# Rikorose/DeepFilterNet

Hardware: NVIDIA H100
Metric: 48kHz audio-sec/sec (batched enhance) (higher is better)
Workload: dtype f32 (bf16x3 tensor-core contractions, fp32 accumulate; DSP and gates IEEE fp32)

## Files before the change

deepfilternet_b200/csrc/dfb_common.cuh:

```cuda
#pragma once
#include <cuda_runtime.h>
#include <stdint.h>

#include <atomic>
#include <cstdarg>
#include <cstdio>
#include <mutex>
#include <string>
#include <vector>

#include "../../include/dfb200.h"

namespace dfb {

extern thread_local std::string g_err;
extern std::atomic<int64_t> g_launches;

inline int fail(int code, const char *fmt, ...) {
    char buf[512];
    va_list ap;
    va_start(ap, fmt);
    vsnprintf(buf, sizeof buf, fmt, ap);
    va_end(ap);
    g_err = buf;
    return code;
}

#define DFB_CUDA(expr)                                                                          \
    do {                                                                                        \
        cudaError_t e__ = (expr);                                                               \
        if (e__ != cudaSuccess)                                                                 \
            return dfb::fail(DFB_ERR_CUDA, "%s failed: %s (%s:%d)", #expr, cudaGetErrorString(e__), \
                             __FILE__, __LINE__);                                               \
    } while (0)

#define DFB_LAUNCH_CHECK()                                                                      \
    do {                                                                                        \
        dfb::g_launches.fetch_add(1, std::memory_order_relaxed);                                \
        cudaError_t e__ = cudaGetLastError();                                                   \
        if (e__ != cudaSuccess)                                                                 \
            return dfb::fail(DFB_ERR_CUDA, "kernel launch failed: %s (%s:%d)",                  \
                             cudaGetErrorString(e__), __FILE__, __LINE__);                      \
    } while (0)

struct ProfScope {
    int slot = -1;
    cudaStream_t s;
    ProfScope(const char *name, cudaStream_t stream);
    ~ProfScope();
};
#define DFB_PROF(name, stream) dfb::ProfScope prof_scope__(name, stream)

struct PerDeviceOnce {
    std::mutex mu;
    std::atomic<unsigned long long> done{0};
    struct Guard {
        std::unique_lock<std::mutex> lk;
        PerDeviceOnce *o = nullptr;
        unsigned long long bit = 0;
        Guard() = default;
        Guard(Guard &&g) noexcept : lk(std::move(g.lk)), o(g.o), bit(g.bit) {}
        explicit operator bool() const { return lk.owns_lock(); }
        ~Guard() { if (lk.owns_lock()) o->done.fetch_or(bit, std::memory_order_release); }
    };
    Guard first() {
        int d = 0;
        cudaGetDevice(&d);
        const unsigned long long bit = 1ull << (d & 63);
        Guard g;
        if (done.load(std::memory_order_acquire) & bit) return g;
        g.lk = std::unique_lock<std::mutex>(mu);
        if (done.load(std::memory_order_acquire) & bit) { g.lk.unlock(); g.lk.release(); return g; }
        g.o = this; g.bit = bit;
        return g;
    }
};

int use_device(int device);

struct Arena {
    char *base = nullptr;
    size_t cap = 0, off = 0;
    int reserve(size_t bytes);
    void reset() { off = 0; }
    template <typename T>
    T *take(size_t n) {
        size_t b = (n * sizeof(T) + 255) & ~size_t(255);
        if (off + b > cap) return nullptr;
        T *p = reinterpret_cast<T *>(base + off);
        off += b;
        return p;
    }
    void release();
};

constexpr int kMaxErb = 64;

struct DspTables {
    const float *window;
    const float2 *tw_a_fwd;
    const float2 *tw_a_inv;
    const float2 *tw960;
    const int *erb_off;
    const float *erb_kinv;
    const unsigned char *band_of_bin;
    float wnorm;
    int fft, hop, F, E;
};

struct RaggedRow { int64_t in_off, len, out_off, out_len, Tf; };

struct LinkRow { int first, n; };
enum { kReduceNone = 0, kReduceMax = 1, kReduceMean = 2 };
struct SlotCtl { float lim, beta, lim0, beta0; int64_t sw; };

__device__ __forceinline__ int stream_first(const int64_t *first, int b, int64_t w0) {
    if (!first) return 0;
    const int64_t d = first[b] - w0;
    return d > 0 ? (int)d : 0;
}

__device__ __forceinline__ float erb_norm_init(int j, int E) {
    return (E == 1) ? -60.f : __fadd_rn(-60.f, __fmul_rn((float)j, __fdiv_rn(-30.f, (float)(E - 1))));
}
__device__ __forceinline__ float unit_norm_init(int k, int Fd) {
    return (Fd == 1) ? 0.001f : __fadd_rn(0.001f, __fmul_rn((float)k, __fdiv_rn(__fsub_rn(0.0001f, 0.001f), (float)(Fd - 1))));
}

struct ApplyParams {
    const float2 *spec;
    const float *m;
    const float *coefs;
    float *audio;
    float2 *spec_out;
    int64_t out_stride;
    int64_t out_offset;
    int64_t out_len;
    int Tf, mode, nb_df, order, lookahead;
    int spec_T, Tv, t_first;
    int mc_T;
    int frames_per_warp;
    int pf, mask_only;
    float pf_beta;
    const float *lsnr;
    float th_min, th_erb, th_df;
    const float *alpha;
    float atten_lim;
    const float *init_tail;
    float *final_tail;
    int carry;
    const RaggedRow *rows;
    int64_t w0;
    int t_emit;
    const int64_t *first;
    const LinkRow *links;
    int reduce;
};

}

struct dfb_state;
namespace dfb {
struct AnaWindow { int t_begin, nf, out_t0, Tbuf; int64_t row_stride; const RaggedRow *rows = nullptr; };
int launch_analysis(dfb_state *st, const float *d_audio, int64_t C, int64_t T, float *d_spec, float *d_erb_db,
                    cudaStream_t s, const float *d_init_mem = nullptr, const AnaWindow *w = nullptr);
int launch_feat_norm(const float *d_erb, int E, int64_t erb_stride, const float *d_spec, int Fd, int64_t spec_stride,
                     int64_t C, int64_t Tf, float alpha, const float *d_erb_state, const float *d_unit_state,
                     float *d_feat_erb, float *d_feat_spec, cudaStream_t s, int64_t Ts = 0, float *d_erb_state_out = nullptr,
                     float *d_unit_state_out = nullptr, bool ref_bits = false);
int launch_apply_synthesis(dfb_state *st, const ApplyParams &p, int64_t B, cudaStream_t s, const SlotCtl *ctl = nullptr);
struct GruWindow { const float *h0; float *hT; int t0, Ts; const int64_t *first = nullptr; int64_t w0 = 0;  };
int launch_gru_tc(cudaStream_t s, const float *xproj, const float *whh, const float *bhh, const float *res, float *hout,
                  unsigned short *hout_hi, unsigned short *hout_lo, int B, int T, long long *dbg = nullptr, int wide = 0,
                  int planes_res = 0, const GruWindow *w = nullptr, int H = 256);
int launch_gemm_bf16x3(cudaStream_t s, const void *x_hi, const void *x_lo, int64_t ldx, const void *w_hi, const void *w_lo,
                       const float *bias, float *y, int64_t ldy, int64_t M, int N, int K);
int launch_gl_bx(cudaStream_t s, const unsigned short *x_hi, const unsigned short *x_lo, int64_t ldx, const float *w_img,
                 const float *res, int64_t ldr, float *y, int64_t ldy, unsigned short *y_hi, unsigned short *y_lo, int64_t ldp,
                 int64_t M, int G, int Ig, int Hg, int act, float oscale, float ooffset);
bool gl_bx_geometry(int G, int Ig, int Hg, int *gpc_out, int *hgp_out, int *stages_out);
int launch_df_convp_tc(cudaStream_t s, const float *c0, const float *w_sw, const float *w2, const float *bias, float *coefs, int B, int T,
                       int Fd, const int64_t *first = nullptr, int64_t w0 = 0);
int launch_to_planes(cudaStream_t s, const float *x, int64_t ldx, int64_t M, int K, unsigned short *hi, unsigned short *lo);
}

struct dfb_state {
    int device, sr, fft, hop, nb_erb, min_nb_erb_freqs;
    std::vector<int64_t> erb;
    std::vector<float> window;
    void *d_tables = nullptr;
    dfb::DspTables tb{};
    dfb::Arena arena;
    cudaStream_t stream = nullptr;
    std::vector<float> analysis_mem, synthesis_mem;
};
```

deepfilternet_b200/csrc/dfb_gl.cu:

```cuda
#include <cuda.h>
#include <cuda_bf16.h>

#include <map>
#include <mutex>
#include <tuple>

#include "dfb_common.cuh"
#include "dfb_ptx.cuh"

namespace dfb {

constexpr int kGxThreads = 288, kGxMaxStages = 6, kGxBoxBytes = 128 * 128 ;
constexpr int kGxMaxChunks = 16;

struct GlBxParams {
    const unsigned short *w_img;
    const float *res; int64_t ldr;
    float *y; int64_t ldy;
    unsigned short *y_hi, *y_lo; int64_t ldp;
    int M, G, Ig, Hg, Hgp, gpc, act, stages;
    float oscale, ooffset;
};

__device__ __forceinline__ float gx_act(float x, int act) {
    if (act == 1) return fmaxf(x, 0.f);
    if (act == 2) return gt_tanh(x);
    return x;
}

__device__ __noinline__ void gl_store_chunk(const GlBxParams &p, int c, int g0, int cpg, int64_t mrow, int lane, float a00, float a01,
                                            float a02, float a03, float a10, float a11, float a12, float a13) {
    const float a[2][4] = {{a00, a01, a02, a03}, {a10, a11, a12, a13}};
    const int gl = c / cpg;
#pragma unroll
    for (int j = 0; j < 2; j++) {
        const int n = (c - gl * cpg) * 16 + j * 8 + 2 * (lane & 3);
        if (n >= p.Hg) continue;
        const int64_t col = (int64_t)(g0 + gl) * p.Hg + n;
        float2 rv[2];
#pragma unroll
        for (int h = 0; h < 2; h++) {
            const int64_t m = mrow + 8 * h;
            rv[h] = (p.res && m < p.M) ? *reinterpret_cast<const float2 *>(p.res + m * p.ldr + col) : make_float2(0.f, 0.f);
        }
#pragma unroll
        for (int h = 0; h < 2; h++) {
            const int64_t m = mrow + 8 * h;
            if (m >= p.M) continue;
            float2 x;
            x.x = gx_act(a[j][2 * h], p.act) * p.oscale + p.ooffset + rv[h].x;
            x.y = gx_act(a[j][2 * h + 1], p.act) * p.oscale + p.ooffset + rv[h].y;
            if (p.y) *reinterpret_cast<float2 *>(p.y + m * p.ldy + col) = x;
            if (p.y_hi) {
                uint32_t hv, lv;
                bf16x2_split(x.x, x.y, hv, lv);
                *reinterpret_cast<uint32_t *>(p.y_hi + m * p.ldp + col) = hv;
                *reinterpret_cast<uint32_t *>(p.y_lo + m * p.ldp + col) = lv;
            }
        }
    }
}

__global__ void __launch_bounds__(kGxThreads, 1)
k_gl_bx(const __grid_constant__ CUtensorMap tmXhi, const __grid_constant__ CUtensorMap tmXlo, const __grid_constant__ GlBxParams p) {
    extern __shared__ __align__(1024) unsigned char gx_smem_raw[];
    const uint32_t sb = (smem_u32(gx_smem_raw) + 1023u) & ~1023u;
    const int warp = threadIdx.x >> 5, lane = threadIdx.x & 31;
    const int slice = blockIdx.x, g0 = slice * p.gpc;
    const int nch = p.gpc * p.Hgp / 16;
    const int cpg = p.Hgp / 16;
    const int nboxes = p.gpc * p.Ig / 64;
    const int ntiles = (p.M + 127) / 128;
    const uint32_t gbytes = (uint32_t)p.Ig * p.Hgp * 2;
    const uint32_t wplane = gbytes * p.gpc;
    const uint32_t lbo = (uint32_t)(p.Hgp / 8) * 128u;
    const uint32_t s_x = sb;
    const uint32_t s_w = s_x + (uint32_t)p.stages * 2 * kGxBoxBytes;
    const uint32_t s_bar = (s_w + 2 * wplane + 127u) & ~127u;
    const uint32_t b_full = s_bar, b_empty = s_bar + 8 * kGxMaxStages, b_w = b_empty + 8 * kGxMaxStages;
    if (threadIdx.x == 0) {
        for (int s = 0; s < p.stages; s++) { mbar_init_a(b_full + 8 * s, 1); mbar_init_a(b_empty + 8 * s, 8); }
        mbar_init_a(b_w, 1);
        fence_barrier_init();
        mbar_expect_tx_a(b_w, 2 * wplane);
        const unsigned char *src = reinterpret_cast<const unsigned char *>(p.w_img);
        bulk_load(s_w, src + (size_t)g0 * gbytes, wplane, b_w);
        bulk_load(s_w + wplane, src + (size_t)p.G * gbytes + (size_t)g0 * gbytes, wplane, b_w);
    }
    __syncthreads();
    if (warp == 8) {
        if (lane == 0) {
            tma_prefetch_desc(&tmXhi); tma_prefetch_desc(&tmXlo);
            const int col0 = g0 * p.Ig;
            int it = 0;
            for (int tile = blockIdx.y; tile < ntiles; tile += gridDim.y)
                for (int b = 0; b < nboxes; b++, it++) {
                    const int s = it % p.stages, n = it / p.stages;
                    if (n > 0) mbar_wait_a(b_empty + 8 * s, (uint32_t)((n - 1) & 1));
                    mbar_expect_tx_a(b_full + 8 * s, 2 * kGxBoxBytes);
                    const uint32_t dst = s_x + (uint32_t)s * 2 * kGxBoxBytes;
                    asm volatile(
                        "cp.async.bulk.tensor.2d.shared::cluster.global.mbarrier::complete_tx::bytes [%0], [%1, {%2, %3}], [%4];"
                        ::"r"(dst), "l"((uint64_t)&tmXhi), "r"(col0 + b * 64), "r"(tile * 128), "r"(b_full + 8 * s) : "memory");
                    asm volatile(
                        "cp.async.bulk.tensor.2d.shared::cluster.global.mbarrier::complete_tx::bytes [%0], [%1, {%2, %3}], [%4];"
                        ::"r"(dst + kGxBoxBytes), "l"((uint64_t)&tmXlo), "r"(col0 + b * 64), "r"(tile * 128), "r"(b_full + 8 * s) : "memory");
                }
        }
        return;
    }
    const int mat = lane >> 3, rr = lane & 7;
    mbar_wait_a(b_w, 0);
    int it = 0;
    for (int tile = blockIdx.y; tile < ntiles; tile += gridDim.y) {
        float acc[kGxMaxChunks][2][4];
#pragma unroll
        for (int c = 0; c < kGxMaxChunks; c++)
#pragma unroll
            for (int e = 0; e < 8; e++) acc[c][e >> 2][e & 3] = 0.f;
        for (int b = 0; b < nboxes; b++, it++) {
            const int s = it % p.stages, n = it / p.stages;
            mbar_wait_a(b_full + 8 * s, (uint32_t)(n & 1));
            const uint32_t xs = s_x + (uint32_t)s * 2 * kGxBoxBytes;
#pragma unroll 1
            for (int k = 0; k < 4; k++) {
                const int col = b * 64 + k * 16;
                const int gl = col / p.Ig, kk = (col - gl * p.Ig) >> 4;
                uint32_t ah[4], al[4];
                const int r = warp * 16 + rr + ((mat & 1) << 3);
                ldsm_x4(xs + sw128_off(r, 2 * k + (mat >> 1)), ah);
                ldsm_x4(xs + kGxBoxBytes + sw128_off(r, 2 * k + (mat >> 1)), al);
                const uint32_t wa = s_w + (uint32_t)gl * gbytes + (uint32_t)(2 * kk + (mat & 1)) * lbo + (uint32_t)rr * 16u;
#pragma unroll
                for (int c = 0; c < kGxMaxChunks; c++) {
                    const int cg = c - gl * cpg;
                    if (c >= nch || cg < 0 || cg >= cpg) continue;
                    const uint32_t o = wa + (uint32_t)(2 * cg + (mat >> 1)) * 128u;
                    uint32_t bh[4], bl[4];
                    ldsm_x4(o, bh);
                    ldsm_x4(o + wplane, bl);
                    mma_bf16x3(acc[c][0], ah, al, bh[0], bh[1], bl[0], bl[1]);
                    mma_bf16x3(acc[c][1], ah, al, bh[2], bh[3], bl[2], bl[3]);
                }
            }
            __syncwarp();
            if (lane == 0) mbar_arrive_a(b_empty + 8 * s);
        }
        const int64_t mrow = (int64_t)tile * 128 + warp * 16 + (lane >> 2);
#pragma unroll
        for (int c = 0; c < kGxMaxChunks; c++)
            if (c < nch)
                gl_store_chunk(p, c, g0, cpg, mrow, lane, acc[c][0][0], acc[c][0][1], acc[c][0][2], acc[c][0][3], acc[c][1][0],
                               acc[c][1][1], acc[c][1][2], acc[c][1][3]);
    }
}

__global__ void __launch_bounds__(256) k_to_planes(const float *__restrict__ x, int64_t ldx, int64_t M, int K,
                                                   unsigned short *__restrict__ hi, unsigned short *__restrict__ lo) {
    const int64_t n4 = M * (K / 4);
    for (int64_t i = (int64_t)blockIdx.x * blockDim.x + threadIdx.x; i < n4; i += (int64_t)gridDim.x * blockDim.x) {
        const int64_t m = i / (K / 4);
        const int k = (int)(i - m * (K / 4)) * 4;
        const float4 v = *reinterpret_cast<const float4 *>(x + m * ldx + k);
        uint32_t h0, l0, h1, l1;
        bf16x2_split(v.x, v.y, h0, l0);
        bf16x2_split(v.z, v.w, h1, l1);
        *reinterpret_cast<uint2 *>(hi + m * K + k) = make_uint2(h0, h1);
        *reinterpret_cast<uint2 *>(lo + m * K + k) = make_uint2(l0, l1);
    }
}

typedef CUresult (*PFN_encodeTiled_gl)(CUtensorMap *, CUtensorMapDataType, cuuint32_t, void *, const cuuint64_t *,
                                       const cuuint64_t *, const cuuint32_t *, const cuuint32_t *, CUtensorMapInterleave,
                                       CUtensorMapSwizzle, CUtensorMapL2promotion, CUtensorMapFloatOOBfill);

int cached_map_bf16(CUtensorMap *out, const void *base, int64_t rows, int64_t cols, int64_t ld, int box_rows) {
    static std::mutex mu;
    static std::map<std::tuple<int, const void *, int64_t, int64_t, int64_t, int>, CUtensorMap> cache;
    static PFN_encodeTiled_gl enc = nullptr;
    int dev = 0;
    cudaGetDevice(&dev);
    std::lock_guard<std::mutex> g(mu);
    auto key = std::make_tuple(dev, base, rows, cols, ld, box_rows);
    auto it = cache.find(key);
    if (it != cache.end()) { *out = it->second; return DFB_OK; }
    if (!enc) {
        void *fp = nullptr;
        cudaDriverEntryPointQueryResult q;
        if (cudaGetDriverEntryPoint("cuTensorMapEncodeTiled", &fp, cudaEnableDefault, &q) != cudaSuccess || q != cudaDriverEntryPointSuccess)
            return fail(DFB_ERR_CUDA, "cuTensorMapEncodeTiled entry point not available");
        enc = (PFN_encodeTiled_gl)fp;
    }
    cuuint64_t dims[2] = {(cuuint64_t)cols, (cuuint64_t)rows};
    cuuint64_t strides[1] = {(cuuint64_t)ld * 2};
    cuuint32_t box[2] = {64u, (cuuint32_t)box_rows};
    cuuint32_t estr[2] = {1, 1};
    CUtensorMap m;
    CUresult r = enc(&m, CU_TENSOR_MAP_DATA_TYPE_BFLOAT16, 2, (void *)base, dims, strides, box, estr, CU_TENSOR_MAP_INTERLEAVE_NONE,
                     CU_TENSOR_MAP_SWIZZLE_128B, CU_TENSOR_MAP_L2_PROMOTION_L2_128B, CU_TENSOR_MAP_FLOAT_OOB_FILL_NONE);
    if (r != CUDA_SUCCESS) return fail(DFB_ERR_CUDA, "cuTensorMapEncodeTiled (bf16) failed (%d)", (int)r);
    if (cache.size() > 4096) cache.clear();
    cache[key] = m;
    *out = m;
    return DFB_OK;
}

int cached_map_f32_sw128(CUtensorMap *out, const void *base, int64_t rows, int64_t cols, int64_t ld, int box_rows) {
    static std::mutex mu;
    static std::map<std::tuple<int, const void *, int64_t, int64_t, int64_t, int>, CUtensorMap> cache;
    static PFN_encodeTiled_gl enc = nullptr;
    int dev = 0;
    cudaGetDevice(&dev);
    std::lock_guard<std::mutex> g(mu);
    auto key = std::make_tuple(dev, base, rows, cols, ld, box_rows);
    auto it = cache.find(key);
    if (it != cache.end()) { *out = it->second; return DFB_OK; }
    if (!enc) {
        void *fp = nullptr;
        cudaDriverEntryPointQueryResult q;
        if (cudaGetDriverEntryPoint("cuTensorMapEncodeTiled", &fp, cudaEnableDefault, &q) != cudaSuccess || q != cudaDriverEntryPointSuccess)
            return fail(DFB_ERR_CUDA, "cuTensorMapEncodeTiled entry point not available");
        enc = (PFN_encodeTiled_gl)fp;
    }
    cuuint64_t dims[2] = {(cuuint64_t)cols, (cuuint64_t)rows};
    cuuint64_t strides[1] = {(cuuint64_t)ld * 4};
    cuuint32_t box[2] = {32u, (cuuint32_t)box_rows};
    cuuint32_t estr[2] = {1, 1};
    CUtensorMap m;
    CUresult r = enc(&m, CU_TENSOR_MAP_DATA_TYPE_FLOAT32, 2, (void *)base, dims, strides, box, estr, CU_TENSOR_MAP_INTERLEAVE_NONE,
                     CU_TENSOR_MAP_SWIZZLE_128B, CU_TENSOR_MAP_L2_PROMOTION_L2_128B, CU_TENSOR_MAP_FLOAT_OOB_FILL_NONE);
    if (r != CUDA_SUCCESS) return fail(DFB_ERR_CUDA, "cuTensorMapEncodeTiled (fp32) failed (%d)", (int)r);
    if (cache.size() > 4096) cache.clear();
    cache[key] = m;
    *out = m;
    return DFB_OK;
}

int launch_to_planes(cudaStream_t s, const float *x, int64_t ldx, int64_t M, int K, unsigned short *hi, unsigned short *lo) {
    if (K % 4 || ldx % 4) return fail(DFB_ERR_UNSUPPORTED, "to_planes: K = %d", K);
    int dev = 0, sms = 0;
    DFB_CUDA(cudaGetDevice(&dev));
    DFB_CUDA(cudaDeviceGetAttribute(&sms, cudaDevAttrMultiProcessorCount, dev));
    DFB_PROF("k_to_planes", s);
    k_to_planes<<<sms * 8, 256, 0, s>>>(x, ldx, M, K, hi, lo);
    DFB_LAUNCH_CHECK();
    return DFB_OK;
}

bool gl_bx_geometry(int G, int Ig, int Hg, int *gpc_out, int *hgp_out, int *stages_out) {
    if (Ig % 16 || Hg % 4 || G < 1) return false;
    const int Hgp = (Hg + 15) / 16 * 16;
    if (Hgp > 256) return false;
    int best = 0;
    for (int gpc = 1; gpc <= G; gpc++) {
        if (G % gpc) continue;
        if (gpc * Hgp > 256 || (gpc * Hgp) % 32) continue;
        if ((gpc * Ig) % 64) continue;
        if ((size_t)gpc * Ig * Hgp * 4 > 100 * 1024) continue;
        best = gpc;
    }
    if (!best) return false;
    const int w = best * Ig * Hgp * 4;
    int stages = (227 * 1024 - 2048 - w - 256) / (2 * kGxBoxBytes);
    if (stages > kGxMaxStages) stages = kGxMaxStages;
    if (stages < 2) return false;
    *gpc_out = best; *hgp_out = Hgp; *stages_out = stages;
    return true;
}

int launch_gl_bx(cudaStream_t s, const unsigned short *x_hi, const unsigned short *x_lo, int64_t ldx, const float *w_img,
                 const float *res, int64_t ldr, float *y, int64_t ldy, unsigned short *y_hi, unsigned short *y_lo, int64_t ldp,
                 int64_t M, int G, int Ig, int Hg, int act, float oscale, float ooffset) {
    int gpc = 0, Hgp = 0, stages = 0;
    if (!gl_bx_geometry(G, Ig, Hg, &gpc, &Hgp, &stages) || M <= 0 || M > 0x7fffffff || (ldx % 8) || ((uintptr_t)x_hi & 15) ||
        ((uintptr_t)x_lo & 15) || (y && ((ldy % 4) || ((uintptr_t)y & 15))) || (res && ((ldr % 4) || ((uintptr_t)res & 15))) ||
        (y_hi && ((ldp % 4) || ((uintptr_t)y_hi & 7) || ((uintptr_t)y_lo & 7))))
        return DFB_ERR_UNSUPPORTED;
    CUtensorMap mh, ml;
    int rc;
    if ((rc = cached_map_bf16(&mh, x_hi, M, (int64_t)G * Ig, ldx, 128)) || (rc = cached_map_bf16(&ml, x_lo, M, (int64_t)G * Ig, ldx, 128)))
        return rc;
    GlBxParams p{reinterpret_cast<const unsigned short *>(w_img), res, ldr, y, ldy, y_hi, y_lo, ldp,
                 (int)M, G, Ig, Hg, Hgp, gpc, act, stages, oscale, ooffset};
    const int smem = 1024 + stages * 2 * kGxBoxBytes + gpc * Ig * Hgp * 4 + 128 + 256;
    static PerDeviceOnce attr_once;
    if (auto once_guard = attr_once.first())
        DFB_CUDA(cudaFuncSetAttribute(k_gl_bx, cudaFuncAttributeMaxDynamicSharedMemorySize, 227 * 1024));
    int dev = 0, sms = 0;
    DFB_CUDA(cudaGetDevice(&dev));
    DFB_CUDA(cudaDeviceGetAttribute(&sms, cudaDevAttrMultiProcessorCount, dev));
    const int slices = G / gpc, ntiles = (int)((M + 127) / 128);
    int groups = sms / slices;
    if (groups < 1) groups = 1;
    if (groups > ntiles) groups = ntiles;
    DFB_PROF("k_gl_bx", s);
    k_gl_bx<<<dim3((unsigned)slices, (unsigned)groups), kGxThreads, smem, s>>>(mh, ml, p);
    DFB_LAUNCH_CHECK();
    return DFB_OK;
}

}
```

deepfilternet_b200/csrc/dfb_model.cu:

```cuda
#include <cuda_bf16.h>

#include <algorithm>
#include <cmath>
#include <cstring>
#include <functional>
#include <map>
#include <numeric>
#include <string>

#include "dfb_common.cuh"
#include "dfb_dwpw.cuh"
#include "dfb_ptx.cuh"

namespace dfb {


enum Act { ACT_NONE = 0, ACT_RELU = 1, ACT_TANH = 2, ACT_SIGMOID = 3 };

__device__ __forceinline__ float act_apply(float x, int act) {
    switch (act) {
        case ACT_RELU: return fmaxf(x, 0.f);
        case ACT_TANH: return tanhf(x);
        case ACT_SIGMOID: return 1.f / (1.f + expf(-x));
        default: return x;
// ... 252 lines not shown
            unsigned short *dh = p.y_hi + m * p.ldy + colbase, *dl = p.y_lo + m * p.ldy + colbase;
            if (nvalid == 4 && (((uintptr_t)dh) & 7) == 0) {
                *reinterpret_cast<uint2 *>(dh) = make_uint2(hi[0] | (uint32_t)hi[1] << 16, hi[2] | (uint32_t)hi[3] << 16);
                *reinterpret_cast<uint2 *>(dl) = make_uint2(lo[0] | (uint32_t)lo[1] << 16, lo[2] | (uint32_t)lo[3] << 16);
            } else {
                for (int j = 0; j < nvalid; j++) { dh[j] = hi[j]; dl[j] = lo[j]; }
            }
        }
    }
}

constexpr int kMaskWarps = 4, kMaskChunk = 8, kMaskLd = kCh + 1;
__global__ void __launch_bounds__(32 * kMaskWarps)
k_mask_out(const float *__restrict__ e0, const float *__restrict__ d1, const float *__restrict__ ps,
           const float *__restrict__ pb, const float *__restrict__ w ,
           const float *__restrict__ bias_p, float *__restrict__ m, int T, int E, int kt,
           const int64_t *__restrict__ first , int64_t w0) {
    extern __shared__ float smem[];
    const int lane = threadIdx.x & 31, warp = threadIdx.x >> 5;
    const int b = blockIdx.y;
    const int t0 = (blockIdx.x * kMaskWarps + warp) * kMaskChunk;
    const int t_first = stream_first(first, b, w0);
    float *buf = smem + warp * 2 * (E + 2) * kMaskLd;
    float *ws = smem + kMaskWarps * 2 * (E + 2) * kMaskLd;
    for (int i = threadIdx.x; i < kt * 3 * kCh; i += blockDim.x) ws[i] = w[i];
    for (int i = lane; i < 2 * (E + 2) * kMaskLd; i += 32) buf[i] = 0.f;
    __syncthreads();
    if (t0 >= T) return;
    const int t1 = min(t0 + kMaskChunk, T);
    const float2 ps2 = *reinterpret_cast<const float2 *>(ps + lane * 2);
    const float2 pb2 = *reinterpret_cast<const float2 *>(pb + lane * 2);
    const float bias = bias_p[0];
    for (int t = (kt > 1 && t0 > 0) ? t0 - 1 : t0; t < t1; t++) {
        float *cur = buf + (t & 1) * (E + 2) * kMaskLd;
        const float *prv = buf + ((t & 1) ^ 1) * (E + 2) * kMaskLd;
        const int64_t base = ((int64_t)b * T + t) * E * kCh;
        for (int f = 0; f < E; f++) {
            float2 e = *reinterpret_cast<const float2 *>(e0 + base + f * kCh + lane * 2);
            float2 d = *reinterpret_cast<const float2 *>(d1 + base + f * kCh + lane * 2);
            cur[(f + 1) * kMaskLd + lane * 2] = fmaxf(e.x * ps2.x + pb2.x, 0.f) + d.x;
            cur[(f + 1) * kMaskLd + lane * 2 + 1] = fmaxf(e.y * ps2.y + pb2.y, 0.f) + d.y;
        }
        __syncwarp();
        if (t >= t0) {
            for (int f = lane; f < E; f += 32) {
                float acc = bias;
                for (int dt = 0; dt < kt; dt++) {
                    const float *src = (dt == kt - 1) ? cur : prv;
                    if (dt != kt - 1 && t <= t_first) continue;
                    for (int df = 0; df < 3; df++) {
                        const float *xr = src + (f + df) * kMaskLd;
                        const float *wr = ws + (dt * 3 + df) * kCh;
#pragma unroll 16
                        for (int c = 0; c < kCh; c++) acc += xr[c] * wr[c];
                    }
                }
                m[((int64_t)b * T + t) * E + f] = sigmoidf_(acc);
            }
        }
        __syncwarp();
    }
}

struct GatherParams {
    const float *src[3]; long long ld[3]; const int *idx[3]; int n;
    float *out; long long ldo;
    unsigned short *hi, *lo; long long ldp;
    int K, relu;
};
__global__ void __launch_bounds__(256) k_gather_sum(GatherParams p) {
    const long long m = blockIdx.x;
    for (int k = threadIdx.x; k < p.K; k += 256) {
        float v = 0.f;
#pragma unroll
        for (int i = 0; i < 3; i++)
            if (i < p.n) v += p.src[i][m * p.ld[i] + p.idx[i][k]];
        if (p.relu) v = fmaxf(v, 0.f);
        if (p.out) p.out[m * p.ldo + k] = v;
        if (p.hi) {
            unsigned short h, l;
            bf16_split(v, h, l);
            p.hi[m * p.ldp + k] = h; p.lo[m * p.ldp + k] = l;
        }
    }
}

template <int O2>
__global__ void __launch_bounds__(128) k_convp_v1(const float *__restrict__ c0, const float *__restrict__ w ,
                                                   const float *__restrict__ bias, float *__restrict__ coefs, long long rows) {
    __shared__ float ws[kCh * O2];
    __shared__ float bs[O2];
    for (int i = threadIdx.x; i < kCh * O2; i += 128) ws[i] = w[i];
    if (threadIdx.x < O2) bs[threadIdx.x] = bias[threadIdx.x];
    __syncthreads();
    const long long r = (long long)blockIdx.x * 128 + threadIdx.x;
    if (r >= rows) return;
    float acc[O2];
#pragma unroll
    for (int k = 0; k < O2; k++) acc[k] = bs[k];
    const float4 *x = reinterpret_cast<const float4 *>(c0 + r * kCh);
#pragma unroll 4
    for (int q = 0; q < kCh / 4; q++) {
        const float4 v = x[q];
#pragma unroll
        for (int k = 0; k < O2; k++)
            acc[k] += v.x * ws[(4 * q) * O2 + k] + v.y * ws[(4 * q + 1) * O2 + k] + v.z * ws[(4 * q + 2) * O2 + k] + v.w * ws[(4 * q + 3) * O2 + k];
    }
    float *o = coefs + r * O2;
#pragma unroll
    for (int k = 0; k < O2; k++) o[k] = tanhf(o[k]) + fmaxf(acc[k], 0.f);
}

constexpr int kMaxO2 = 16;

}

using namespace dfb;


struct GruChunk { float *h; bool have_state; int t0; int Bs; const int64_t *first; int64_t w0; };

struct dfb_model {
    int device;
    dfb_model_config cfg;
    std::map<std::string, std::pair<float *, int64_t>> t;
    std::map<std::string, std::pair<const float *, int64_t>> dbg;
    float *slab = nullptr;
    long long *gru_dbg = nullptr;
    Arena arena;
    int dev_chunks = 0, host_chunks = 4, n_lanes = 2;
    int post_filter = 0, mask_only = 0;
    float pf_beta = 0.02f;
    size_t max_workspace = size_t(40) << 30;
    std::vector<int64_t> erb_widths;
    Arena aux_arena;
    cudaStream_t stream = nullptr;
    cudaStream_t h2d = nullptr, d2h = nullptr;
    struct Lane {
        cudaStream_t main = nullptr, hi = nullptr, aux = nullptr, dhi = nullptr, daux = nullptr, low = nullptr;
        cudaEvent_t ev_fork = nullptr, ev_join = nullptr, ev_fork_enc = nullptr, ev_join_enc = nullptr, ev_in = nullptr,
                    ev_out = nullptr, ev_c0 = nullptr, ev_convp = nullptr, ev_skip = nullptr, ev_done = nullptr;
    } lanes[2];
    Arena arena1;
    const float *get(const std::string &n) const {
        auto it = t.find(n);
        return it == t.end() ? nullptr : it->second.first;
    }
};

static int need(const dfb_model *m, const char *name, int64_t numel, const float **out) {
    auto it = m->t.find(name);
    if (it == m->t.end()) return fail(DFB_ERR_INVALID, "missing weight tensor '%s'", name);
    if (numel >= 0 && it->second.second != numel)
        return fail(DFB_ERR_INVALID, "weight tensor '%s' has %lld elements, expected %lld", name,
                    (long long)it->second.second, (long long)numel);
    *out = it->second.first;
    return DFB_OK;
}

extern "C" int dfb_model_create(dfb_model **out, int device, const dfb_model_config *cfg, const dfb_tensor *tensors,
                                int n_tensors, const int64_t *erb_widths) {
    if (!out || !cfg || !tensors) return fail(DFB_ERR_INVALID, "null argument");
    *out = nullptr;
    if (cfg->conv_ch != kCh) return fail(DFB_ERR_UNSUPPORTED, "conv_ch = %d (built kernels: 64)", cfg->conv_ch);
    if (cfg->model_kind < 1 || cfg->model_kind > 3) return fail(DFB_ERR_UNSUPPORTED, "model_kind %d", cfg->model_kind);
    if (cfg->model_kind == 1 && (cfg->emb_hidden != cfg->df_hidden || cfg->emb_hidden != cfg->nb_erb / 4 * kCh || cfg->conv_kt != 2 ||
                                 cfg->inp_kt != 2 || cfg->df_order != 5))
        return fail(DFB_ERR_UNSUPPORTED, "DeepFilterNet v1: only the shipped topology is built (hidden = conv_ch * nb_erb / 4, kt 2, order 5)");
    if (cfg->conv_kt < 1 || cfg->conv_kt > 2 || cfg->inp_kt < 1 || cfg->inp_kt > 3)
        return fail(DFB_ERR_UNSUPPORTED, "conv kernel time taps (%d, %d) unsupported", cfg->conv_kt, cfg->inp_kt);
    if ((cfg->emb_hidden != 256 && cfg->emb_hidden != 512) || (cfg->df_hidden != 256 && cfg->df_hidden != 512))
        return fail(DFB_ERR_UNSUPPORTED, "GRU hidden sizes (%d, %d): built kernels cover 256 and 512", cfg->emb_hidden,
                    cfg->df_hidden);
    if (cfg->nb_erb % 8 || cfg->nb_erb > 64 || cfg->nb_df % 8 || cfg->nb_df > 128 || 2 * cfg->df_order > kMaxO2)
        return fail(DFB_ERR_UNSUPPORTED, "nb_erb / nb_df / df_order outside the built kernels");
    int rc = use_device(device);
    if (rc) return rc;
    dfb_model *m = new dfb_model();
    m->device = device;
    m->cfg = *cfg;
    if (erb_widths) m->erb_widths.assign(erb_widths, erb_widths + cfg->nb_erb);
    if (const char *e = getenv("DFB_DEVICE_CHUNKS")) m->dev_chunks = atoi(e) > 0 ? atoi(e) : 0;
    if (const char *e = getenv("DFB_HOST_CHUNKS")) m->host_chunks = atoi(e) > 0 ? atoi(e) : 1;
    if (const char *e = getenv("DFB_LANES")) m->n_lanes = atoi(e) == 1 ? 1 : 2;
    if (const char *e = getenv("DFB_MAX_WORKSPACE_MB")) {
        const long long mb = atoll(e);
        if (mb > 0) m->max_workspace = (size_t)mb << 20;
    }
    size_t total = 0;
    for (int i = 0; i < n_tensors; i++) total += ((size_t)tensors[i].numel * 4 + 255) & ~size_t(255);
    if (cudaMalloc(&m->slab, total + 256) != cudaSuccess) {
        delete m;
        return fail(DFB_ERR_OOM, "cudaMalloc(%zu) for weights failed", total);
    }
    size_t off = 0;
    std::vector<float> tmp;
    for (int i = 0; i < n_tensors; i++) {
        const dfb_tensor &tt = tensors[i];
        if (!tt.name || !tt.data || tt.numel <= 0) { dfb_model_free(m); return fail(DFB_ERR_INVALID, "bad tensor %d", i); }
        float *dst = (float *)((char *)m->slab + off);
        if (cudaMemcpy(dst, tt.data, (size_t)tt.numel * 4, cudaMemcpyHostToDevice) != cudaSuccess) {
            dfb_model_free(m);
            return fail(DFB_ERR_CUDA, "weight upload failed");
        }
        m->t[tt.name] = {dst, tt.numel};
        off += ((size_t)tt.numel * 4 + 255) & ~size_t(255);
    }
    int prio_least = 0, prio_greatest = 0;
    cudaDeviceGetStreamPriorityRange(&prio_least, &prio_greatest);
    int prio_enc = prio_greatest + 1;
    if (prio_enc > prio_least) prio_enc = prio_least;
    bool ok = cudaStreamCreateWithFlags(&m->stream, cudaStreamNonBlocking) == cudaSuccess &&
              cudaStreamCreateWithFlags(&m->h2d, cudaStreamNonBlocking) == cudaSuccess &&
              cudaStreamCreateWithFlags(&m->d2h, cudaStreamNonBlocking) == cudaSuccess;
    for (auto &L : m->lanes) {
        ok = ok && cudaStreamCreateWithPriority(&L.main, cudaStreamNonBlocking, prio_enc) == cudaSuccess &&
             cudaStreamCreateWithPriority(&L.hi, cudaStreamNonBlocking, prio_enc) == cudaSuccess &&
             cudaStreamCreateWithPriority(&L.aux, cudaStreamNonBlocking, prio_enc) == cudaSuccess &&
             cudaStreamCreateWithPriority(&L.dhi, cudaStreamNonBlocking, prio_greatest) == cudaSuccess &&
             cudaStreamCreateWithPriority(&L.daux, cudaStreamNonBlocking, prio_greatest) == cudaSuccess &&
             cudaStreamCreateWithPriority(&L.low, cudaStreamNonBlocking, prio_least) == cudaSuccess;
        for (cudaEvent_t *e : {&L.ev_fork, &L.ev_join, &L.ev_fork_enc, &L.ev_join_enc, &L.ev_in, &L.ev_out, &L.ev_c0, &L.ev_convp,
                               &L.ev_skip, &L.ev_done})
            ok = ok && cudaEventCreateWithFlags(e, cudaEventDisableTiming) == cudaSuccess;
    }
    if (!ok) {
        dfb_model_free(m);
        return fail(DFB_ERR_CUDA, "stream creation failed");
    }
    *out = m;
    return DFB_OK;
}

extern "C" void dfb_model_free(dfb_model *m) {
    if (!m) return;
    cudaSetDevice(m->device);
    m->arena.release();
    m->arena1.release();
    m->aux_arena.release();
    if (m->h2d) cudaStreamDestroy(m->h2d);
    if (m->d2h) cudaStreamDestroy(m->d2h);
    if (m->slab) cudaFree(m->slab);
    if (m->stream) cudaStreamDestroy(m->stream);
    for (auto &L : m->lanes) {
        for (cudaStream_t st : {L.main, L.hi, L.aux, L.dhi, L.daux, L.low})
            if (st) cudaStreamDestroy(st);
        for (cudaEvent_t e : {L.ev_fork, L.ev_join, L.ev_fork_enc, L.ev_join_enc, L.ev_in, L.ev_out, L.ev_c0, L.ev_convp, L.ev_skip, L.ev_done})
            if (e) cudaEventDestroy(e);
    }
    delete m;
}

extern "C" int dfb_debug_gru_timing(dfb_model *m, int steps, long long *h_out) {
    if (!m) return fail(DFB_ERR_INVALID, "null model");
    cudaSetDevice(m->device);
    if (h_out && m->gru_dbg) {
        DFB_CUDA(cudaDeviceSynchronize());
        DFB_CUDA(cudaMemcpy(h_out, m->gru_dbg, sizeof(long long) * 8 * steps, cudaMemcpyDeviceToHost));
    }
    if (m->gru_dbg) { cudaFree(m->gru_dbg); m->gru_dbg = nullptr; }
    if (steps > 0 && !h_out) {
        DFB_CUDA(cudaMalloc(&m->gru_dbg, sizeof(long long) * 8 * steps));
        DFB_CUDA(cudaMemset(m->gru_dbg, 0, sizeof(long long) * 8 * steps));
    }
    return DFB_OK;
}

extern "C" int64_t dfb_model_debug_fetch(dfb_model *m, const char *name, float *h_out, int64_t max_numel) {
    if (!m || !name || !h_out) return fail(DFB_ERR_INVALID, "null argument");
    auto it = m->dbg.find(name);
    if (it == m->dbg.end()) return fail(DFB_ERR_INVALID, "no activation named '%s'", name);
    int64_t n = it->second.second < max_numel ? it->second.second : max_numel;
    cudaSetDevice(m->device);
    if (cudaDeviceSynchronize() != cudaSuccess ||
        cudaMemcpy(h_out, it->second.first, (size_t)n * 4, cudaMemcpyDeviceToHost) != cudaSuccess)
        return fail(DFB_ERR_CUDA, "debug fetch failed: %s", cudaGetErrorString(cudaGetLastError()));
    return n;
}

extern "C" int64_t dfb_model_workspace_bytes(const dfb_model *m) { return m ? (int64_t)m->arena.cap : 0; }

namespace {

int run_gl(cudaStream_t s, const float *x, int64_t ldx, const float *w, const float *bias, const float *res,
           int64_t ldr, float *y, int64_t ldy, int64_t M, int G, int I, int Hh, int act, float oscale = 1.f,
           float ooffset = 0.f, unsigned short *y_hi = nullptr, unsigned short *y_lo = nullptr) {
    GlParams p{x, ldx, w, bias, res, ldr, y, ldy, M, G, I / G, Hh / G, act, oscale, ooffset, y_hi, y_lo};
    if ((p.Ig % 4) || (ldx % 4)) return fail(DFB_ERR_UNSUPPORTED, "grouped linear: K not a multiple of 4");
    if (G > 1 && (p.Hg % 4)) return fail(DFB_ERR_UNSUPPORTED, "grouped linear: group width %d not a multiple of 4", p.Hg);
    int tiles = (p.Hg + kGlBN - 1) / kGlBN;
    int gpc = (p.Hg < kGlBN && kGlBN % p.Hg == 0) ? (kGlBN / p.Hg < G ? kGlBN / p.Hg : G) : 1;
    dim3 grid((unsigned)((M + kGlBM - 1) / kGlBM), (unsigned)(((G + gpc - 1) / gpc) * tiles));
    static const bool detail = getenv("DFB_PROF_DETAIL") && atoi(getenv("DFB_PROF_DETAIL"));
    char name[64];
    if (detail) snprintf(name, sizeof name, "k_grouped_linear[%dx%d/%d]", I, Hh, G);
    else snprintf(name, sizeof name, "%s", p.G == 1 && p.bias && p.Hg >= 512 ? "k_grouped_linear[gru_proj]" : "k_grouped_linear");
    DFB_PROF(name, s);
    k_grouped_linear<<<grid, 256, 0, s>>>(p);
    DFB_LAUNCH_CHECK();
    return DFB_OK;
}

int run_gru(dfb_model *m, cudaStream_t s, const char *name, int layers, int H, int in_dim, const float *res_last, float *y,
            float *xproj, float *tmp_h, int B, int T, const unsigned short *x_hi, const unsigned short *x_lo,
            unsigned short *pl_hi, unsigned short *pl_lo, int wide, unsigned short *out_hi, unsigned short *out_lo,
            bool *out_planes_ok, const GruChunk *ck) {
    if (out_planes_ok) *out_planes_ok = false;
    if (!x_hi || !x_lo || !pl_hi || !pl_lo || in_dim % 64)
        return fail(DFB_ERR_INVALID, "GRU '%s': input planes, scratch planes and an input width that is a multiple of 64 are required", name);
    const int t0 = ck ? ck->t0 : 0, Tn = T - t0;
    const int64_t M = (int64_t)B * T;
    int cur_dim = in_dim;
    const unsigned short *cur_hi = x_hi, *cur_lo = x_lo;
    for (int l = 0; l < layers; l++) {
        std::string base = std::string(name) + ".l" + std::to_string(l);
        const float *w_hh, *b_ih, *b_hh, *w_hi, *w_lo;
        int rc;
        if ((rc = need(m, (base + ".w_hh").c_str(), (int64_t)3 * H * H, &w_hh))) return rc;
        if ((rc = need(m, (base + ".b_ih").c_str(), 3 * H, &b_ih))) return rc;
        if ((rc = need(m, (base + ".b_hh").c_str(), 3 * H, &b_hh))) return rc;
        if ((rc = need(m, (base + ".w_ih_hi").c_str(), (int64_t)3 * H * cur_dim / 2, &w_hi)) ||
            (rc = need(m, (base + ".w_ih_lo").c_str(), (int64_t)3 * H * cur_dim / 2, &w_lo)))
            return rc;
        if ((rc = launch_gemm_bf16x3(s, cur_hi, cur_lo, cur_dim, w_hi, w_lo, b_ih, xproj, 3 * H, M, 3 * H, cur_dim))) return rc;
        const bool last = l == layers - 1;
        float *dst = last ? y : tmp_h;
        float *hs = ck && ck->h ? ck->h + (int64_t)l * ck->Bs * H : nullptr;
        GruWindow gw{ck && ck->have_state ? hs : nullptr, hs, t0, T, ck ? ck->first : nullptr, ck ? ck->w0 : 0};
        unsigned short *hi = last ? out_hi : pl_hi, *lo = last ? out_lo : pl_lo;
        if ((rc = launch_gru_tc(s, xproj, w_hh, b_hh, last ? res_last : nullptr, dst, hi, lo, B, Tn, m->gru_dbg,
                                wide, last ? 1 : 0, &gw, H)))
            return rc;
        if (last && hi && out_planes_ok) *out_planes_ok = true;
        cur_hi = pl_hi; cur_lo = pl_lo;
        cur_dim = H;
    }
    return DFB_OK;
}

}
namespace dfb {
template <int MODE>
int launch_dwpw_tc(cudaStream_t s, DwPwParams p, const float *w_sw, int B);
}
namespace {

template <int MODE>
int run_dwpw(cudaStream_t s, DwPwParams p, int B, const float *w_sw = nullptr) {
    if (w_sw) return launch_dwpw_tc<MODE>(s, p, w_sw, B);
    static PerDeviceOnce attr_once;
    const int smem = (kCh * kCh + 128 * kLdA) * 4;
    if (auto once_guard = attr_once.first()) {
        DFB_CUDA(cudaFuncSetAttribute(k_dwpw<MODE>, cudaFuncAttributeMaxDynamicSharedMemorySize, smem));
    }
    p.NF = 128 / p.Fout;
    if (p.NF < 1) p.NF = 1;
    if (p.NF * p.Fout > 128 || (p.NF * p.Fout) % 4) return fail(DFB_ERR_UNSUPPORTED, "dwpw tile: Fout = %d", p.Fout);
    dim3 grid((unsigned)((p.T + p.NF - 1) / p.NF), (unsigned)B);
    DFB_PROF("k_dwpw", s);
    k_dwpw<MODE><<<grid, 256, smem, s>>>(p);
    DFB_LAUNCH_CHECK();
    return DFB_OK;
}

}

struct FwdBufs {
    float *e0, *e1, *e2, *e3, *c0, *c1, *emb_in, *emb, *g_a, *g_b, *g_h, *xproj, *dec_emb, *d3, *d2, *d1, *dfc;
    unsigned short *ga_hi, *ga_lo, *gh_hi, *gh_lo;
    float *g_a2, *g_h2, *xproj2, *dfskip;
    unsigned short *ga2_hi, *ga2_lo, *gh2_hi, *gh2_lo;
    unsigned short *c1_hi, *c1_lo, *embin_hi, *embin_lo, *gb_hi, *gb_lo, *emb_hi, *emb_lo, *dfc_hi, *dfc_lo;
};

struct FwdBufsV1 {
    float *e0, *e1, *e2, *e3, *c0, *c1, *c1g, *cemb, *emb, *xproj, *xproj2, *y[3], *embo, *dec_old, *dec, *p3, *p2, *p1, *p0, *d3, *d2, *d1,
        *z[2], *dfc;
    unsigned short *emb_hi, *emb_lo, *y_hi[3], *y_lo[3], *embo_hi, *embo_lo, *z_hi[2], *z_lo[2], *dfc_hi, *dfc_lo, *scr_hi, *scr_lo;
};
static size_t fwd_plan_v1(const dfb_model_config &c, size_t M, Arena *a, FwdBufsV1 *f) {
    const int E = c.nb_erb, Fd = c.nb_df, H = c.emb_hidden;
    size_t bytes = 0;
    auto take = [&](size_t n) -> float * {
        bytes += (n * 4 + 255) & ~size_t(255);
        return a ? a->take<float>(n) : nullptr;
    };
    auto take16 = [&](size_t n) { return reinterpret_cast<unsigned short *>(take((n + 1) / 2)); };
    FwdBufsV1 t{};
    t.e0 = take(M * E * kCh); t.e1 = take(M * (E / 2) * kCh); t.e2 = take(M * (E / 4) * kCh); t.e3 = take(M * (E / 4) * kCh);
    t.c0 = take(M * Fd * kCh); t.c1 = take(M * (Fd / 2) * kCh); t.c1g = take(M * (Fd / 2) * kCh);
    t.cemb = take(M * H); t.emb = take(M * H); t.xproj = take(M * 3 * H); t.xproj2 = take(M * 3 * H);
    for (int i = 0; i < 3; i++) { t.y[i] = take(M * H); t.y_hi[i] = take16(M * H); t.y_lo[i] = take16(M * H); }
    for (int i = 0; i < 2; i++) { t.z[i] = take(M * H); t.z_hi[i] = take16(M * H); t.z_lo[i] = take16(M * H); }
    t.embo = take(M * H); t.dec_old = take(M * H); t.dec = take(M * H); t.dfc = take(M * H);
    t.p3 = take(M * (E / 4) * kCh); t.p2 = take(M * (E / 4) * kCh); t.p1 = take(M * (E / 2) * kCh); t.p0 = take(M * E * kCh);
    t.d3 = take(M * (E / 4) * kCh); t.d2 = take(M * (E / 2) * kCh); t.d1 = take(M * E * kCh);
    t.emb_hi = take16(M * H); t.emb_lo = take16(M * H); t.embo_hi = take16(M * H); t.embo_lo = take16(M * H);
    t.dfc_hi = take16(M * H); t.dfc_lo = take16(M * H); t.scr_hi = take16(M * H); t.scr_lo = take16(M * H);
    if (f) *f = t;
    return bytes + 4096;
}

static size_t fwd_plan(const dfb_model_config &c, size_t M, Arena *a, FwdBufs *f) {
    if (c.model_kind == 1 && !a) return fwd_plan_v1(c, M, nullptr, nullptr);
    const int E = c.nb_erb, Fd = c.nb_df, H = c.emb_hidden, Hd = c.df_hidden;
    const int ED = E / 4 * kCh;
    const int emb_in_dim = c.enc_concat ? 2 * ED : ED;
    const int emb_dim = c.model_kind == 2 ? H : ED;
    const int Hmax = H > Hd ? H : Hd;
    size_t bytes = 0;
    auto take = [&](size_t n) -> float * {
        bytes += (n * 4 + 255) & ~size_t(255);
        return a ? a->take<float>(n) : nullptr;
    };
    FwdBufs t{};
    t.e0 = take(M * E * kCh); t.e1 = take(M * (E / 2) * kCh); t.e2 = take(M * (E / 4) * kCh);
    t.emb_in = take(M * emb_in_dim);
    t.e3 = c.enc_concat ? t.emb_in : take(M * ED);
    t.c0 = take(M * Fd * kCh); t.c1 = take(M * (Fd / 2) * kCh);
    t.emb = take(M * emb_dim);
    t.g_a = take(M * Hmax); t.g_b = take(M * Hmax); t.g_h = take(M * Hmax);
    t.xproj = take(M * 3 * Hmax);
    t.dec_emb = take(M * ED); t.d3 = take(M * ED); t.d2 = take(M * (E / 2) * kCh);
    t.d1 = take(M * E * kCh); t.dfc = take(M * Hmax);
    t.ga_hi = reinterpret_cast<unsigned short *>(take(M * Hmax / 2)); t.ga_lo = reinterpret_cast<unsigned short *>(take(M * Hmax / 2));
    t.gh_hi = reinterpret_cast<unsigned short *>(take(M * Hmax / 2)); t.gh_lo = reinterpret_cast<unsigned short *>(take(M * Hmax / 2));
    t.g_a2 = take(M * Hmax); t.g_h2 = take(M * Hmax); t.xproj2 = take(M * 3 * Hmax); t.dfskip = take(M * Hmax);
    t.ga2_hi = reinterpret_cast<unsigned short *>(take(M * Hmax / 2)); t.ga2_lo = reinterpret_cast<unsigned short *>(take(M * Hmax / 2));
    t.gh2_hi = reinterpret_cast<unsigned short *>(take(M * Hmax / 2)); t.gh2_lo = reinterpret_cast<unsigned short *>(take(M * Hmax / 2));
    auto take16 = [&](size_t n) { return reinterpret_cast<unsigned short *>(take((n + 1) / 2)); };
    t.c1_hi = take16(M * (Fd / 2) * kCh); t.c1_lo = take16(M * (Fd / 2) * kCh);
    t.embin_hi = take16(M * emb_in_dim); t.embin_lo = take16(M * emb_in_dim);
    t.gb_hi = take16(M * Hmax); t.gb_lo = take16(M * Hmax);
    t.emb_hi = take16(M * emb_dim); t.emb_lo = take16(M * emb_dim);
    t.dfc_hi = take16(M * Hmax); t.dfc_lo = take16(M * Hmax);
    if (f) *f = t;
    return bytes + 4096;
}

struct ChunkCtx {
    int Rc;
    int Tsx, Tx;
    float *h_enc, *h_erb, *h_df;
    bool have_state;
    float *dec_tail;
    int dec_tail_n;
    int lane;
    cudaEvent_t wait_dec;
    int Bs;
    const RaggedRow *rows;
    int64_t W0;
    const int64_t *first;
};
constexpr int kHalo = 8;

static int forward_impl(dfb_model *m, Arena &arena, const float *d_feat_erb, const float *d_feat_spec, int B, int T,
                        float *d_m, float *d_coefs, float *d_lsnr, float *d_alpha, cudaStream_t s, ChunkCtx *cx = nullptr);

extern "C" int dfb_model_forward(dfb_model *m, const float *d_feat_erb, const float *d_feat_spec, int64_t B64,
                                 int64_t T64, float *d_m, float *d_coefs, float *d_lsnr, float *d_alpha,
                                 void *stream) {
    if (!m || !d_feat_erb || !d_feat_spec || !d_m || !d_coefs) return fail(DFB_ERR_INVALID, "null argument");
    if (B64 <= 0 || T64 <= 0) return DFB_OK;
    if (B64 > 65535) return fail(DFB_ERR_INVALID, "more than 65535 streams per call");
    DFB_CUDA(cudaSetDevice(m->device));
    int rc = m->arena.reserve(fwd_plan(m->cfg, (size_t)B64 * T64, nullptr, nullptr));
    if (rc) return rc;
    m->arena.reset();
    rc = forward_impl(m, m->arena, d_feat_erb, d_feat_spec, (int)B64, (int)T64, d_m, d_coefs, d_lsnr, d_alpha,
                      (cudaStream_t)stream);
    m->arena.reset();
    return rc;
}

static int forward_body(dfb_model *m, Arena &arena, const float *d_feat_erb, const float *d_feat_spec, int B, int T,
                        float *d_m, float *d_coefs, float *d_lsnr, float *d_alpha, cudaStream_t s_in, ChunkCtx *cx);

static int forward_v1(dfb_model *m, Arena &arena, const float *d_feat_erb, const float *d_feat_spec, int B, int T,
                      float *d_m, float *d_coefs, float *d_lsnr, float *d_alpha, cudaStream_t s_in, ChunkCtx *cx);

static int forward_impl(dfb_model *m, Arena &arena, const float *d_feat_erb, const float *d_feat_spec, int B, int T,
                        float *d_m, float *d_coefs, float *d_lsnr, float *d_alpha, cudaStream_t s_in, ChunkCtx *cx) {
    const int rc = m->cfg.model_kind == 1
        ? forward_v1(m, arena, d_feat_erb, d_feat_spec, B, T, d_m, d_coefs, d_lsnr, d_alpha, s_in, cx)
        : forward_body(m, arena, d_feat_erb, d_feat_spec, B, T, d_m, d_coefs, d_lsnr, d_alpha, s_in, cx);
    if (rc) cudaDeviceSynchronize();
    return rc;
}

static int forward_body(dfb_model *m, Arena &arena, const float *d_feat_erb, const float *d_feat_spec, int B, int T,
                        float *d_m, float *d_coefs, float *d_lsnr, float *d_alpha, cudaStream_t s_in, ChunkCtx *cx) {
    const dfb_model_config &c = m->cfg;
    const int Tsx = cx ? cx->Tsx : T, Tx = cx ? cx->Tx : T;
    const RaggedRow *rows = cx ? cx->rows : nullptr;
    const int64_t W0 = cx ? cx->W0 : 0;
    const int64_t *first = cx ? cx->first : nullptr;
    GruChunk ck_enc{cx ? cx->h_enc : nullptr, cx && cx->have_state, cx ? cx->Rc : 0, cx ? cx->Bs : B, first, W0};
    GruChunk ck_erb{cx ? cx->h_erb : nullptr, cx && cx->have_state, cx ? cx->Rc : 0, cx ? cx->Bs : B, first, W0};
    GruChunk ck_df{cx ? cx->h_df : nullptr, cx && cx->have_state, cx ? cx->Rc : 0, cx ? cx->Bs : B, first, W0};
    static const bool serial = getenv("DFB_SERIAL") && atoi(getenv("DFB_SERIAL"));
    dfb_model::Lane &L = m->lanes[cx ? cx->lane : 0];
    cudaStream_t s = serial ? s_in : L.hi;
    cudaStream_t sl = serial ? s_in : L.low;
    if (!serial) {
        DFB_CUDA(cudaEventRecord(L.ev_in, s_in));
        DFB_CUDA(cudaStreamWaitEvent(s, L.ev_in, 0));
    }
    auto finish = [&]() -> int {
        DFB_CUDA(cudaStreamWaitEvent(s, L.ev_join, 0));
        if (!serial) {
            DFB_CUDA(cudaEventRecord(L.ev_out, s));
            DFB_CUDA(cudaStreamWaitEvent(s_in, L.ev_out, 0));
        }
        return DFB_OK;
    };
    const int64_t M = (int64_t)B * T;
    const int E = c.nb_erb, Fd = c.nb_df, H = c.emb_hidden, Hd = c.df_hidden;
    const int ED = E / 4 * kCh;
    const int emb_in_dim = c.enc_concat ? 2 * ED : ED;
    const int emb_dim = c.model_kind == 2 ? H : ED;
    int rc;
    FwdBufs f{};
    fwd_plan(c, (size_t)M, &arena, &f);
    if (!f.gh2_lo || !f.dfskip || !f.dfc_lo) return fail(DFB_ERR_OOM, "forward workspace exhausted for %lld frames", (long long)M);
    m->dbg.clear();
    m->dbg["e0"] = {f.e0, M * E * kCh}; m->dbg["e1"] = {f.e1, M * (E / 2) * kCh}; m->dbg["e2"] = {f.e2, M * (E / 4) * kCh};
    m->dbg["e3"] = {f.e3, c.enc_concat ? M * emb_in_dim : M * ED}; m->dbg["c0"] = {f.c0, M * Fd * kCh};
    m->dbg["c1"] = {f.c1, M * (Fd / 2) * kCh}; m->dbg["emb_in"] = {f.emb_in, M * emb_in_dim};
    m->dbg["emb"] = {f.emb, M * emb_dim}; m->dbg["dec_emb"] = {f.dec_emb, M * ED}; m->dbg["d3"] = {f.d3, M * ED};
    m->dbg["d2"] = {f.d2, M * (E / 2) * kCh}; m->dbg["d1"] = {f.d1, M * E * kCh}; m->dbg["dfc"] = {f.dfc, M * Hd};
    m->dbg["g_a"] = {f.g_a, M * (H > Hd ? H : Hd)}; m->dbg["g_b"] = {f.g_b, M * (H > Hd ? H : Hd)};
    m->dbg["xproj"] = {f.xproj, M * 3 * (H > Hd ? H : Hd)};
    const int64_t e3_fs = c.enc_concat ? 2 * ED : ED;
    struct Pl { unsigned short *hi, *lo; int64_t ld; bool ok; };
    Pl pl_c1{f.c1_hi, f.c1_lo, (int64_t)Fd / 2 * kCh, false}, pl_embin{f.embin_hi, f.embin_lo, emb_in_dim, false},
       pl_gb{f.gb_hi, f.gb_lo, H, false}, pl_emb{f.emb_hi, f.emb_lo, emb_dim, false}, pl_dfc{f.dfc_hi, f.dfc_lo, Hd, false},
       pl_ga{f.ga_hi, f.ga_lo, H, false}, pl_ga2{f.ga2_hi, f.ga2_lo, Hd, false};
    auto ensure_planes = [&](cudaStream_t st, const float *x, int64_t ldx, int K, Pl &pl) -> int {
        if (pl.ok) return DFB_OK;
        if (pl.ld != K) return fail(DFB_ERR_INVALID, "plane pitch mismatch");
        int r = launch_to_planes(st, x, ldx, M, K, pl.hi, pl.lo);
        if (!r) pl.ok = true;
        return r;
    };
    auto gl = [&](cudaStream_t st, const char *wname, const float *x, int64_t ldx, Pl *xin, int G, int I, int Hh, int act,
                  const float *res, int64_t ldr, float *y, int64_t ldy, Pl *yout, int64_t ycol = 0) -> int {
        const float *w;
        int r;
        if ((r = need(m, wname, (int64_t)I * Hh / G, &w))) return r;
        unsigned short *yh = yout ? yout->hi + ycol : nullptr, *yl = yout ? yout->lo + ycol : nullptr;
        const std::string bx = std::string(wname) + "_bx";
        int gpc, hgp, stages;
        if (xin && m->get(bx) && gl_bx_geometry(G, I / G, Hh / G, &gpc, &hgp, &stages)) {
            if ((r = ensure_planes(st, x, ldx, I, *xin))) return r;
            r = launch_gl_bx(st, xin->hi, xin->lo, xin->ld, m->get(bx), res, ldr, y, ldy, yh, yl, yout ? yout->ld : 0, M, G, I / G,
                             Hh / G, act, 1.f, 0.f);
            if (r != DFB_ERR_UNSUPPORTED) {
                if (!r && yout) yout->ok = true;
                return r;
            }
        }
        const bool ffma_planes = yout && yout->ld == ldy;
        r = run_gl(st, x, ldx, w, nullptr, res, ldr, y, ldy, M, G, I, Hh, act, 1.f, 0.f, ffma_planes ? yh : nullptr, ffma_planes ? yl : nullptr);
        if (!r && yout) yout->ok = ffma_planes;
        return r;
    };

    {
        const float *w, *bb;
        if ((rc = need(m, "enc.erb_conv0.w", c.inp_kt * 3 * kCh, &w)) || (rc = need(m, "enc.erb_conv0.b", kCh, &bb))) return rc;
        dim3 grid((unsigned)((T + kInFrames - 1) / kInFrames), (unsigned)B);
        int smem = (kInFrames + c.inp_kt - 1) * (E + 2) * 4;
        DFB_PROF("k_conv_in[erb_conv0]", s);
        k_conv_in<1><<<grid, 256, smem, s>>>(d_feat_erb, w, bb, f.e0, T, E, c.inp_kt, c.conv_lookahead, Tsx, Tx, 0, rows, W0, first);
        DFB_LAUNCH_CHECK();
    }
    const float *pw_sw = nullptr;
    auto blk = [&](const char *name, DwPwParams &p) -> int {
        std::string n(name);
        int r;
        if ((r = need(m, (n + ".dw").c_str(), -1, &p.dw)) || (r = need(m, (n + ".b").c_str(), kCh, &p.bias)) ||
            (r = need(m, (n + ".pw_sw").c_str(), kCh * kCh, &pw_sw)))
            return r;
        return DFB_OK;
    };
    cudaStream_t sa = serial ? s : L.aux;
    DFB_CUDA(cudaEventRecord(L.ev_fork_enc, s));
    DFB_CUDA(cudaStreamWaitEvent(sa, L.ev_fork_enc, 0));
    auto mk = [&](const float *in, int Fin, int64_t in_fs, float *out, int Fout, int64_t out_fs, int kt) {
        DwPwParams p{};
        p.in = in; p.Fin = Fin; p.in_fs = in_fs; p.out = out; p.Fout = Fout; p.out_fs = out_fs; p.kt = kt; p.T = T;
        p.lookahead = 0;
        p.first = first; p.w0 = W0;
        return p;
    };
    {
        DwPwParams p{};
        {
            const float *w, *bb;
            if ((rc = need(m, "enc.df_conv0.w", c.inp_kt * 3 * 2 * kCh, &w)) || (rc = need(m, "enc.df_conv0.b", kCh, &bb))) return rc;
            dim3 grid((unsigned)((T + kInFrames - 1) / kInFrames), (unsigned)B);
            int smem = (kInFrames + c.inp_kt - 1) * (Fd + 2) * 2 * 4;
            DFB_PROF("k_conv_in[df_conv0]", sa);
            k_conv_in<2><<<grid, 256, smem, sa>>>(d_feat_spec, w, bb, f.c0, T, Fd, c.inp_kt, c.conv_lookahead, Tsx, Tx, 0, rows, W0, first);
            DFB_LAUNCH_CHECK();
            DFB_CUDA(cudaEventRecord(L.ev_c0, sa));
        }
        p = mk(f.c0, Fd, (int64_t)Fd * kCh, f.c1, Fd / 2, (int64_t)Fd / 2 * kCh, c.conv_kt);
        if ((rc = blk("enc.df_conv1", p))) return rc;
        p.out = nullptr; p.out_hi = pl_c1.hi; p.out_lo = pl_c1.lo; pl_c1.ok = true;
        m->dbg.erase("c1");
        if ((rc = run_dwpw<DW_S2>(sa, p, B, pw_sw))) return rc;
        DFB_CUDA(cudaEventRecord(L.ev_join_enc, sa));
        DFB_CUDA(cudaStreamWaitEvent(sl, L.ev_c0, 0));
        const int O2 = 2 * c.df_order;
        if (c.df_order != 5 || c.df_pathway_kt != 5)
            return fail(DFB_ERR_UNSUPPORTED, "df_order %d / df_pathway_kernel_size_t %d (built kernels: 5, 5)", c.df_order,
                        c.df_pathway_kt);
        if (Fd % 2) return fail(DFB_ERR_UNSUPPORTED, "df pathway conv: odd nb_df");
        const float *w_sw, *w2, *bb;
        if ((rc = need(m, "df_dec.df_convp.w_sw", kCh * kCh, &w_sw)) || (rc = need(m, "df_dec.df_convp.w2", O2 * O2, &w2)) ||
            (rc = need(m, "df_dec.df_convp.b", O2, &bb)))
            return rc;
        if ((rc = launch_df_convp_tc(sl, f.c0, w_sw, w2, bb, d_coefs, B, T, Fd, first, W0))) return rc;
        DFB_CUDA(cudaEventRecord(L.ev_convp, sl));
    }
    {
        DwPwParams p = mk(f.e0, E, (int64_t)E * kCh, f.e1, E / 2, (int64_t)E / 2 * kCh, c.conv_kt);
        if ((rc = blk("enc.erb_conv1", p)) || (rc = run_dwpw<DW_S2>(s, p, B, pw_sw))) return rc;
        p = mk(f.e1, E / 2, (int64_t)E / 2 * kCh, f.e2, E / 4, (int64_t)E / 4 * kCh, c.conv_kt);
        if ((rc = blk("enc.erb_conv2", p)) || (rc = run_dwpw<DW_S2>(s, p, B, pw_sw))) return rc;
        p = mk(f.e2, E / 4, (int64_t)E / 4 * kCh, f.e3, E / 4, e3_fs, c.conv_kt);
        if ((rc = blk("enc.erb_conv3", p))) return rc;
        if (c.enc_concat) { p.out_hi = pl_embin.hi; p.out_lo = pl_embin.lo; }
        if ((rc = run_dwpw<DW_S1>(s, p, B, pw_sw))) return rc;

    }
    DFB_CUDA(cudaStreamWaitEvent(s, L.ev_join_enc, 0));
    {
        const int I = Fd / 2 * kCh;
        if (c.enc_concat) {
            rc = gl(s, "enc.df_fc_emb.gl", f.c1, I, &pl_c1, c.g_df_fc_emb, I, ED, ACT_RELU, nullptr, 0, f.emb_in + ED, emb_in_dim,
                    &pl_embin, ED);
        } else {
            rc = gl(s, "enc.df_fc_emb.gl", f.c1, I, &pl_c1, c.g_df_fc_emb, I, ED, ACT_RELU, f.e3, ED, f.emb_in, emb_in_dim, &pl_embin);
        }
        if (rc) return rc;
    }
    {
        if ((rc = gl(s, "enc.emb_gru.in.gl", f.emb_in, emb_in_dim, &pl_embin, c.g_enc_in, emb_in_dim, H, ACT_RELU, nullptr, 0, f.g_a, H,
                     &pl_ga))) return rc;
        float *gout = c.g_enc_out ? f.g_b : f.emb;
        Pl &pl_gout = c.g_enc_out ? pl_gb : pl_emb;
        if ((rc = run_gru(m, s, "enc.emb_gru", c.enc_gru_layers, H, H, nullptr, gout, f.xproj, f.g_h, B, T, f.ga_hi, f.ga_lo,
                          f.gh_hi, f.gh_lo, 0, pl_gout.hi, pl_gout.lo, &pl_gout.ok, cx ? &ck_enc : nullptr))) return rc;
        if (c.g_enc_out) {
            if ((rc = gl(s, "enc.emb_gru.out.gl", f.g_b, H, &pl_gb, c.g_enc_out, H, ED, ACT_RELU, nullptr, 0, f.emb, emb_dim, &pl_emb)))
                return rc;
        }
        if ((rc = ensure_planes(s, f.emb, emb_dim, emb_dim, pl_emb))) return rc;
        if (d_lsnr) {
            const float *lw, *lb;
            if ((rc = need(m, "enc.lsnr.w", emb_dim, &lw)) || (rc = need(m, "enc.lsnr.b", 1, &lb))) return rc;
            if ((rc = run_gl(s, f.emb, emb_dim, lw, lb, nullptr, 0, d_lsnr, 1, M, 1, emb_dim, 1, ACT_SIGMOID, c.lsnr_scale, c.lsnr_offset))) return rc;
        }
    }
    DFB_CUDA(cudaEventRecord(L.ev_fork, s));
    if (!serial) { s = L.dhi; sa = L.daux; DFB_CUDA(cudaStreamWaitEvent(s, L.ev_fork, 0)); }
    DFB_CUDA(cudaStreamWaitEvent(sa, L.ev_fork, 0));
    if (cx && cx->wait_dec) {
        DFB_CUDA(cudaStreamWaitEvent(s, cx->wait_dec, 0));
        DFB_CUDA(cudaStreamWaitEvent(sa, cx->wait_dec, 0));
    }
    static const char *wide_env = getenv("DFB_WIDE_BRANCH");
    const int wide_df = !wide_env || !strcmp(wide_env, "df") || !strcmp(wide_env, "both");
    const int wide_erb = wide_env && (!strcmp(wide_env, "erb") || !strcmp(wide_env, "both"));
    const bool early_skip = c.g_df_skip && c.model_kind != 2;
    if (early_skip) {
        if ((rc = gl(s, "df_dec.df_skip.gl", f.emb, emb_dim, &pl_emb, c.g_df_skip, emb_dim, Hd, ACT_NONE, nullptr, 0, f.dfskip, Hd, nullptr)))
            return rc;
        DFB_CUDA(cudaEventRecord(L.ev_skip, s));
    }
    {
        cudaStream_t s = sa;
        if ((rc = gl(s, "df_dec.df_gru.in.gl", f.emb, emb_dim, &pl_emb, c.g_df_in, emb_dim, Hd, ACT_RELU, nullptr, 0, f.g_a2, Hd, &pl_ga2)))
            return rc;
        const float *res = c.model_kind == 2 ? f.g_a2 : (early_skip ? f.dfskip : nullptr);
        if (early_skip) DFB_CUDA(cudaStreamWaitEvent(s, L.ev_skip, 0));
        if ((rc = run_gru(m, s, "df_dec.df_gru", c.df_gru_layers, Hd, Hd, res, f.dfc, f.xproj2, f.g_h2, B, T, f.ga2_hi, f.ga2_lo,
                          f.gh2_hi, f.gh2_lo, wide_df, pl_dfc.hi, pl_dfc.lo, &pl_dfc.ok, cx ? &ck_df : nullptr))) return rc;
        if (c.g_df_skip && !early_skip) {
            if ((rc = gl(s, "df_dec.df_skip.gl", f.emb, emb_dim, &pl_emb, c.g_df_skip, emb_dim, Hd, ACT_NONE, f.dfc, Hd, f.dfc, Hd, nullptr)))
                return rc;
            pl_dfc.ok = false;
        }
        if (d_alpha && c.model_kind == 2) {
            const float *aw, *ab;
            if ((rc = need(m, "df_dec.df_fc_a.w", Hd, &aw)) || (rc = need(m, "df_dec.df_fc_a.b", 1, &ab))) return rc;
            if ((rc = run_gl(s, f.dfc, Hd, aw, ab, nullptr, 0, d_alpha, 1, M, 1, Hd, 1, ACT_SIGMOID))) return rc;
        }
        const int O2 = 2 * c.df_order;
        DFB_CUDA(cudaStreamWaitEvent(s, L.ev_convp, 0));
        if ((rc = gl(s, "df_dec.df_out.gl", f.dfc, Hd, &pl_dfc, c.g_df_out, Hd, Fd * O2, ACT_TANH, d_coefs, (int64_t)Fd * O2, d_coefs,
                     (int64_t)Fd * O2, nullptr))) return rc;
    }
    DFB_CUDA(cudaEventRecord(L.ev_join, sa));
    {
        if ((rc = gl(s, "erb_dec.emb_gru.in.gl", f.emb, emb_dim, &pl_emb, c.g_erb_in, emb_dim, H, ACT_RELU, nullptr, 0, f.g_a, H, &pl_ga)))
            return rc;
        const float *res = c.model_kind == 2 ? f.g_a : nullptr;
        pl_gb.ok = false;
        if ((rc = run_gru(m, s, "erb_dec.emb_gru", c.erb_gru_layers, H, H, res, f.g_b, f.xproj, f.g_h, B, T, f.ga_hi, f.ga_lo,
                          f.gh_hi, f.gh_lo, wide_erb, pl_gb.hi, pl_gb.lo, &pl_gb.ok, cx ? &ck_erb : nullptr))) return rc;
        if ((rc = gl(s, "erb_dec.emb_gru.out.gl", f.g_b, H, &pl_gb, c.g_erb_out, H, ED, ACT_RELU, nullptr, 0, f.dec_emb, ED, nullptr)))
            return rc;
        if (cx && cx->dec_tail && c.conv_kt > 1) {
            const size_t fb = sizeof(float) * ED;
            const int nl = cx->Rc < cx->dec_tail_n ? cx->Rc : cx->dec_tail_n;
            if (cx->have_state && nl > 0)
                DFB_CUDA(cudaMemcpy2DAsync(f.dec_emb + (size_t)(cx->Rc - nl) * ED, fb * T, cx->dec_tail + (size_t)(kHalo - nl) * ED,
                                           fb * kHalo, fb * nl, B, cudaMemcpyDeviceToDevice, s));
            const int ns = T < kHalo ? T : kHalo;
            DFB_CUDA(cudaMemcpy2DAsync(cx->dec_tail + (size_t)(kHalo - ns) * ED, fb * kHalo, f.dec_emb + (size_t)(T - ns) * ED, fb * T,
                                       fb * ns, B, cudaMemcpyDeviceToDevice, s));
            cx->dec_tail_n = ns;
        }
        auto path = [&](DwPwParams &p, const char *pn, const float *pt, int64_t pfs) -> int {
            std::string n(pn);
            p.path = pt; p.path_fs = pfs;
            int r;
            if ((r = need(m, (n + ".s").c_str(), kCh, &p.ps)) || (r = need(m, (n + ".b").c_str(), kCh, &p.pb))) return r;
            return DFB_OK;
        };
        DwPwParams p = mk(f.dec_emb, E / 4, ED, f.d3, E / 4, ED, c.conv_kt);
        if ((rc = blk("erb_dec.convt3", p)) || (rc = path(p, "erb_dec.conv3p", f.e3, e3_fs)) || (rc = run_dwpw<DW_S1>(s, p, B, pw_sw))) return rc;
        p = mk(f.d3, E / 4, ED, f.d2, E / 2, (int64_t)E / 2 * kCh, 1);
        if ((rc = blk("erb_dec.convt2", p)) || (rc = path(p, "erb_dec.conv2p", f.e2, (int64_t)E / 4 * kCh)) || (rc = run_dwpw<DW_T2>(s, p, B, pw_sw))) return rc;
        const float *ps, *pb, *w, *bb;
        if ((rc = need(m, "erb_dec.conv0p.s", kCh, &ps)) || (rc = need(m, "erb_dec.conv0p.b", kCh, &pb)) ||
            (rc = need(m, "erb_dec.conv0_out.w", c.conv_kt * 3 * kCh, &w)) || (rc = need(m, "erb_dec.conv0_out.b", 1, &bb)))
            return rc;
        p = mk(f.d2, E / 2, (int64_t)E / 2 * kCh, f.d1, E, (int64_t)E * kCh, 1);
        if ((rc = blk("erb_dec.convt1", p)) || (rc = path(p, "erb_dec.conv1p", f.e1, (int64_t)E / 2 * kCh))) return rc;
        const bool fused_mask = c.conv_kt == 1 && 128 % E == 0;
        if (fused_mask) {
            p.mk_e0 = f.e0; p.mk_ps = ps; p.mk_pb = pb; p.mk_w = w; p.mk_bias = bb; p.mk_out = d_m;
            p.out = nullptr;
            m->dbg.erase("d1");
        }
        if ((rc = run_dwpw<DW_T2>(s, p, B, pw_sw))) return rc;
        if (fused_mask) return finish();
        static PerDeviceOnce attr_once;
        int smem = (kMaskWarps * 2 * (E + 2) * kMaskLd + c.conv_kt * 3 * kCh) * 4;
        if (auto once_guard = attr_once.first()) {
            DFB_CUDA(cudaFuncSetAttribute(k_mask_out, cudaFuncAttributeMaxDynamicSharedMemorySize,
                                          (kMaskWarps * 2 * (64 + 2) * kMaskLd + 2 * 3 * kCh) * 4));
        }
        int per_cta = kMaskWarps * kMaskChunk;
        dim3 grid((unsigned)((T + per_cta - 1) / per_cta), (unsigned)B);
        DFB_PROF("k_mask_out", s);
        k_mask_out<<<grid, 32 * kMaskWarps, smem, s>>>(f.e0, f.d1, ps, pb, w, bb, d_m, T, E, c.conv_kt, first, W0);
        DFB_LAUNCH_CHECK();
    }
    return finish();
}

static int forward_v1(dfb_model *m, Arena &arena, const float *d_feat_erb, const float *d_feat_spec, int B, int T,
                      float *d_m, float *d_coefs, float *d_lsnr, float *d_alpha, cudaStream_t s_in, ChunkCtx *cx) {
    const dfb_model_config &c = m->cfg;
    if (cx && (cx->Rc != 0 || cx->have_state)) return fail(DFB_ERR_UNSUPPORTED, "DeepFilterNet v1 runs as one window per signal");
    const int Tsx = cx ? cx->Tsx : T, Tx = cx ? cx->Tx : T;
    static const bool serial = getenv("DFB_SERIAL") && atoi(getenv("DFB_SERIAL"));
    dfb_model::Lane &L = m->lanes[cx ? cx->lane : 0];
    cudaStream_t s = serial ? s_in : L.hi, sa = serial ? s_in : L.aux;
    if (!serial) {
        DFB_CUDA(cudaEventRecord(L.ev_in, s_in));
        DFB_CUDA(cudaStreamWaitEvent(s, L.ev_in, 0));
    }
    const int64_t M = (int64_t)B * T;
    const int E = c.nb_erb, Fd = c.nb_df, H = c.emb_hidden, O2 = 2 * c.df_order, kt = c.conv_kt;
    int rc;
    FwdBufsV1 f{};
    fwd_plan_v1(c, (size_t)M, &arena, &f);
    if (!f.scr_lo) return fail(DFB_ERR_OOM, "forward workspace exhausted for %lld frames", (long long)M);
    m->dbg.clear();
    m->dbg["e0"] = {f.e0, M * E * kCh}; m->dbg["e1"] = {f.e1, M * (E / 2) * kCh}; m->dbg["e2"] = {f.e2, M * (E / 4) * kCh};
    m->dbg["e3"] = {f.e3, M * (E / 4) * kCh}; m->dbg["c0"] = {f.c0, M * Fd * kCh}; m->dbg["c1"] = {f.c1, M * (Fd / 2) * kCh};
    m->dbg["cemb"] = {f.cemb, M * H}; m->dbg["emb_in"] = {f.emb, M * H}; m->dbg["emb"] = {f.embo, M * H};
    m->dbg["dec_emb"] = {f.dec, M * H}; m->dbg["d3"] = {f.d3, M * (E / 4) * kCh}; m->dbg["d2"] = {f.d2, M * (E / 2) * kCh};
    m->dbg["d1"] = {f.d1, M * E * kCh}; m->dbg["dfc"] = {f.dfc, M * H}; m->dbg["y0"] = {f.y[0], M * H};
    const float *ones, *zeros;
    if ((rc = need(m, "v1.ones", kCh, &ones)) || (rc = need(m, "v1.zeros", kCh, &zeros))) return rc;
    auto table = [&](const char *name, int n, const int **out) -> int {
        const float *t;
        int r = need(m, name, n, &t);
        *out = reinterpret_cast<const int *>(t);
        return r;
    };
    const int *idx_c1, *idx_e3, *idx_shuf, *idx_id, *idx_dec, *idx_gshuf;
    if ((rc = table("v1.idx_c1", Fd / 2 * kCh, &idx_c1)) || (rc = table("v1.idx_e3", H, &idx_e3)) || (rc = table("v1.idx_shuf", H, &idx_shuf)) ||
        (rc = table("v1.idx_id", H, &idx_id)) || (rc = table("v1.idx_dec", H, &idx_dec)) || (rc = table("v1.idx_gshuf", H, &idx_gshuf)))
        return rc;
    auto gather = [&](cudaStream_t st, int n, const float *const *src, const int64_t *ld, const int *const *idx, int K, int relu,
                      float *out, unsigned short *hi, unsigned short *lo) -> int {
        GatherParams g{};
        for (int i = 0; i < n; i++) { g.src[i] = src[i]; g.ld[i] = ld[i]; g.idx[i] = idx[i]; }
        g.n = n; g.out = out; g.ldo = K; g.hi = hi; g.lo = lo; g.ldp = K; g.K = K; g.relu = relu;
        DFB_PROF("k_gather_sum", st);
        k_gather_sum<<<(unsigned)M, 256, 0, st>>>(g);
        DFB_LAUNCH_CHECK();
        return DFB_OK;
    };
    auto block = [&](cudaStream_t st, const char *name, int mode, const float *in, int Fin, float *out, int Fout, int bkt, int la,
                     const float *path) -> int {
        DwPwParams p{};
        std::string n(name);
        int r;
        if ((r = need(m, (n + ".dw").c_str(), bkt * 3 * kCh, &p.dw)) || (r = need(m, (n + ".pw").c_str(), kCh * kCh, &p.pw)) ||
            (r = need(m, (n + ".b").c_str(), kCh, &p.bias)))
            return r;
        p.in = in; p.Fin = Fin; p.in_fs = (int64_t)Fin * kCh; p.out = out; p.Fout = Fout; p.out_fs = (int64_t)Fout * kCh; p.kt = bkt; p.T = T;
        p.lookahead = la;
        if (path) { p.path = path; p.path_fs = p.in_fs; p.ps = ones; p.pb = zeros; }
        const float *w_sw = nullptr;
        if (la == 0 && !(mode == DW_T2 && bkt != 1) && (r = need(m, (n + ".pw_sw").c_str(), kCh * kCh, &w_sw))) return r;
        if (mode == DW_S1) return run_dwpw<DW_S1>(st, p, B, w_sw);
        if (mode == DW_S2) return run_dwpw<DW_S2>(st, p, B, w_sw);
        return run_dwpw<DW_T2>(st, p, B, w_sw);
    };
    DFB_CUDA(cudaEventRecord(L.ev_fork_enc, s));
    DFB_CUDA(cudaStreamWaitEvent(sa, L.ev_fork_enc, 0));
    {
        const float *w, *bb;
        if ((rc = need(m, "enc.erb_conv0.w", c.inp_kt * 3 * kCh, &w)) || (rc = need(m, "enc.erb_conv0.b", kCh, &bb))) return rc;
        dim3 grid((unsigned)((T + kInFrames - 1) / kInFrames), (unsigned)B);
        const int la = c.conv_lookahead > 0 ? 1 : 0;
        {
            DFB_PROF("k_conv_in[erb_conv0]", s);
            k_conv_in<1><<<grid, 256, (kInFrames + c.inp_kt - 1) * (E + 2) * 4, s>>>(d_feat_erb, w, bb, f.e0, T, E, c.inp_kt, la, Tsx, Tx, -la,
                                                                                      nullptr, 0, nullptr);
            DFB_LAUNCH_CHECK();
        }
        if ((rc = need(m, "enc.df_conv0.w", c.inp_kt * 3 * 2 * kCh, &w)) || (rc = need(m, "enc.df_conv0.b", kCh, &bb))) return rc;
        DFB_PROF("k_conv_in[df_conv0]", sa);
        k_conv_in<2><<<grid, 256, (kInFrames + c.inp_kt - 1) * (Fd + 2) * 2 * 4, sa>>>(d_feat_spec, w, bb, f.c0, T, Fd, c.inp_kt, c.conv_lookahead,
                                                                                      Tsx, Tx, -c.conv_lookahead, nullptr, 0, nullptr);
        DFB_LAUNCH_CHECK();
    }
    if ((rc = block(sa, "enc.df_conv1", DW_S2, f.c0, Fd, f.c1, Fd / 2, kt, 0, nullptr))) return rc;
    {
        const float *src[1] = {f.c1}; const int64_t ld[1] = {(int64_t)Fd / 2 * kCh}; const int *ix[1] = {idx_c1};
        if ((rc = gather(sa, 1, src, ld, ix, Fd / 2 * kCh, 0, f.c1g, nullptr, nullptr))) return rc;
        const float *w, *bb;
        const int I = Fd / 2 * kCh;
        if ((rc = need(m, "enc.df_fc_emb.gl", (int64_t)I * H / c.g_df_fc_emb, &w)) || (rc = need(m, "enc.df_fc_emb.bias", H, &bb))) return rc;
        if ((rc = run_gl(sa, f.c1g, I, w, bb, nullptr, 0, f.cemb, H, M, c.g_df_fc_emb, I, H, ACT_NONE))) return rc;
    }
    DFB_CUDA(cudaEventRecord(L.ev_join_enc, sa));
    if ((rc = block(s, "enc.erb_conv1", DW_S2, f.e0, E, f.e1, E / 2, kt, c.conv_lookahead > 1 ? 1 : 0, nullptr)) ||
        (rc = block(s, "enc.erb_conv2", DW_S2, f.e1, E / 2, f.e2, E / 4, kt, c.conv_lookahead > 2 ? 1 : 0, nullptr)) ||
        (rc = block(s, "enc.erb_conv3", DW_S1, f.e2, E / 4, f.e3, E / 4, kt, 0, nullptr)))
        return rc;
    DFB_CUDA(cudaStreamWaitEvent(s, L.ev_join_enc, 0));
    {
        const float *src[2] = {f.e3, f.cemb}; const int64_t ld[2] = {H, H}; const int *ix[2] = {idx_e3, idx_shuf};
        if ((rc = gather(s, 2, src, ld, ix, H, 0, f.emb, f.emb_hi, f.emb_lo))) return rc;
    }
    auto ggru = [&](cudaStream_t st, const char *name, int layers, unsigned short *x_hi, unsigned short *x_lo, float **y,
                    unsigned short **y_hi, unsigned short **y_lo, float *xproj, float *hbase, float *out, unsigned short *out_hi,
                    unsigned short *out_lo) -> int {
        unsigned short *ch = x_hi, *cl = x_lo;
        for (int l = 0; l < layers; l++) {
            const std::string nm = std::string(name) + ".g" + std::to_string(l);
            GruChunk ck{hbase ? hbase + (int64_t)l * B * H : nullptr, false, 0, B, nullptr, 0};
            bool ok = false;
            int r = run_gru(m, st, nm.c_str(), 1, H, H, nullptr, y[l], xproj, nullptr, B, T, ch, cl, f.scr_hi, f.scr_lo, 0, y_hi[l], y_lo[l], &ok,
                            hbase ? &ck : nullptr);
            if (r) return r;
            ch = y_hi[l]; cl = y_lo[l];
        }
        const float *src[3]; int64_t ld[3]; const int *ix[3];
        for (int l = 0; l < layers; l++) { src[l] = y[l]; ld[l] = H; ix[l] = l == layers - 1 ? idx_id : idx_gshuf; }
        return gather(st, layers, src, ld, ix, H, 0, out, out_hi, out_lo);
    };
    if (c.enc_gru_layers > 3 || c.df_gru_layers > 2) return fail(DFB_ERR_UNSUPPORTED, "DeepFilterNet v1: more GRU layers than built (3 / 2)");
    if ((rc = ggru(s, "enc.emb_gru", c.enc_gru_layers, f.emb_hi, f.emb_lo, f.y, f.y_hi, f.y_lo, f.xproj, cx ? cx->h_enc : nullptr, f.embo,
                   f.embo_hi, f.embo_lo)))
        return rc;
    if (d_lsnr) {
        const float *lw, *lb;
        if ((rc = need(m, "enc.lsnr.w", H, &lw)) || (rc = need(m, "enc.lsnr.b", 1, &lb))) return rc;
        if ((rc = run_gl(s, f.embo, H, lw, lb, nullptr, 0, d_lsnr, 1, M, 1, H, 1, ACT_SIGMOID, c.lsnr_scale, c.lsnr_offset))) return rc;
    }
    DFB_CUDA(cudaEventRecord(L.ev_fork, s));
    if (!serial) { s = L.dhi; sa = L.daux; DFB_CUDA(cudaStreamWaitEvent(s, L.ev_fork, 0)); }
    DFB_CUDA(cudaStreamWaitEvent(sa, L.ev_fork, 0));
    {
        if ((rc = ggru(sa, "df_dec.df_gru", c.df_gru_layers, f.embo_hi, f.embo_lo, f.z, f.z_hi, f.z_lo, f.xproj2, cx ? cx->h_df : nullptr, f.dfc,
                       f.dfc_hi, f.dfc_lo)))
            return rc;
        if (d_alpha) {
            const float *aw, *ab;
            if ((rc = need(m, "df_dec.df_fc_a.w", H, &aw)) || (rc = need(m, "df_dec.df_fc_a.b", 1, &ab))) return rc;
            if ((rc = run_gl(sa, f.dfc, H, aw, ab, nullptr, 0, d_alpha, 1, M, 1, H, 1, ACT_SIGMOID))) return rc;
        }
        const float *w_t, *bb, *w_hi, *w_lo;
        const int N = Fd * O2;
        if ((rc = need(m, "df_dec.df_fc_out.w_t", (int64_t)H * N, &w_t)) || (rc = need(m, "df_dec.df_fc_out.b", N, &bb))) return rc;
        rc = DFB_ERR_UNSUPPORTED;
        if (m->get("df_dec.df_fc_out.w_hi")) {
            if ((rc = need(m, "df_dec.df_fc_out.w_hi", (int64_t)H * N / 2, &w_hi)) || (rc = need(m, "df_dec.df_fc_out.w_lo", (int64_t)H * N / 2, &w_lo))) return rc;
            rc = launch_gemm_bf16x3(sa, f.dfc_hi, f.dfc_lo, H, w_hi, w_lo, bb, d_coefs, N, M, N, H);
        }
        if (rc == DFB_ERR_UNSUPPORTED) rc = run_gl(sa, f.dfc, H, w_t, bb, nullptr, 0, d_coefs, N, M, 1, H, N, ACT_NONE);
        if (rc) return rc;
        const float *pw, *pb;
        if ((rc = need(m, "df_dec.df_convp.w", kCh * O2, &pw)) || (rc = need(m, "df_dec.df_convp.b", O2, &pb))) return rc;
        const long long rows = (long long)M * Fd;
        DFB_PROF("k_convp_v1", sa);
        k_convp_v1<10><<<(unsigned)((rows + 127) / 128), 128, 0, sa>>>(f.c0, pw, pb, d_coefs, rows);
        DFB_LAUNCH_CHECK();
    }
    DFB_CUDA(cudaEventRecord(L.ev_join, sa));
    {
        const float *w, *bb;
        if ((rc = need(m, "erb_dec.fc_emb.gl", (int64_t)H * H / c.g_erb_in, &w)) || (rc = need(m, "erb_dec.fc_emb.bias", H, &bb))) return rc;
        if ((rc = run_gl(s, f.embo, H, w, bb, nullptr, 0, f.dec_old, H, M, c.g_erb_in, H, H, ACT_RELU))) return rc;
        const float *src[1] = {f.dec_old}; const int64_t ld[1] = {H}; const int *ix[1] = {idx_dec};
        if ((rc = gather(s, 1, src, ld, ix, H, 0, f.dec, nullptr, nullptr))) return rc;
        if ((rc = block(s, "erb_dec.conv3p", DW_S1, f.e3, E / 4, f.p3, E / 4, 1, 0, nullptr)) ||
            (rc = block(s, "erb_dec.conv2p", DW_S1, f.e2, E / 4, f.p2, E / 4, 1, 0, nullptr)) ||
            (rc = block(s, "erb_dec.conv1p", DW_S1, f.e1, E / 2, f.p1, E / 2, 1, 0, nullptr)) ||
            (rc = block(s, "erb_dec.conv0p", DW_S1, f.e0, E, f.p0, E, 1, 0, nullptr)))
            return rc;
        if ((rc = block(s, "erb_dec.convt3", DW_S1, f.dec, E / 4, f.d3, E / 4, kt, 0, f.p3)) ||
            (rc = block(s, "erb_dec.convt2", DW_T2, f.d3, E / 4, f.d2, E / 2, kt, 0, f.p2)) ||
            (rc = block(s, "erb_dec.convt1", DW_T2, f.d2, E / 2, f.d1, E, kt, 0, f.p1)))
            return rc;
        if ((rc = need(m, "erb_dec.conv0_out.w", kt * 3 * kCh, &w)) || (rc = need(m, "erb_dec.conv0_out.b", 1, &bb))) return rc;
        static PerDeviceOnce attr_once;
        const int smem = (kMaskWarps * 2 * (E + 2) * kMaskLd + kt * 3 * kCh) * 4;
        if (auto once_guard = attr_once.first()) {
            DFB_CUDA(cudaFuncSetAttribute(k_mask_out, cudaFuncAttributeMaxDynamicSharedMemorySize, (kMaskWarps * 2 * (64 + 2) * kMaskLd + 2 * 3 * kCh) * 4));
        }
        const int per_cta = kMaskWarps * kMaskChunk;
        dim3 grid((unsigned)((T + per_cta - 1) / per_cta), (unsigned)B);
        DFB_PROF("k_mask_out", s);
        k_mask_out<<<grid, 32 * kMaskWarps, smem, s>>>(f.p0, f.d1, ones, zeros, w, bb, d_m, T, E, kt, nullptr, 0);
        DFB_LAUNCH_CHECK();
    }
    DFB_CUDA(cudaStreamWaitEvent(s, L.ev_join, 0));
    if (!serial) {
        DFB_CUDA(cudaEventRecord(L.ev_out, s));
        DFB_CUDA(cudaStreamWaitEvent(s_in, L.ev_out, 0));
    }
    return DFB_OK;
}

extern "C" int dfb_model_set_chunking(dfb_model *m, int device_chunks, int host_chunks, int lanes) {
    if (!m || device_chunks < 0 || host_chunks < 1 || lanes < 1 || lanes > 2) return fail(DFB_ERR_INVALID, "bad chunking parameters");
    m->dev_chunks = device_chunks; m->host_chunks = host_chunks; m->n_lanes = lanes;
    return DFB_OK;
}

static int check_state(const dfb_model *m, const dfb_state *st) {
    if (m->device != st->device) return fail(DFB_ERR_INVALID, "model and state live on different devices");
    if (st->tb.E != m->cfg.nb_erb)
        return fail(DFB_ERR_INVALID, "DF state has %d ERB bands, the model was built for %d", st->tb.E, m->cfg.nb_erb);
    if (!m->erb_widths.empty())
        for (int i = 0; i < m->cfg.nb_erb; i++)
            if (m->erb_widths[i] != st->erb[i])
                return fail(DFB_ERR_INVALID, "DF state's ERB band %d is %lld bins wide, the model was built for %lld", i,
                            (long long)st->erb[i], (long long)m->erb_widths[i]);
    return DFB_OK;
}

static int apply_mode(const dfb_model *m) { return m->cfg.model_kind == 3 ? 1 : 2; }
static void apply_options(const dfb_model *m, dfb::ApplyParams &p) {
    p.pf = m->post_filter; p.pf_beta = m->pf_beta; p.mask_only = m->mask_only;
}

extern "C" int dfb_model_set_options(dfb_model *m, int post_filter, float pf_beta, int mask_only) {
    if (!m) return fail(DFB_ERR_INVALID, "null model");
    m->post_filter = post_filter ? 1 : 0;
    m->pf_beta = pf_beta;
    m->mask_only = mask_only ? 1 : 0;
    return DFB_OK;
}

static int apply_impl(dfb_model *m, dfb_state *st, const float *d_spec, const float *d_m, const float *d_coefs, const float *d_alpha,
                      int64_t B, int64_t T, float *d_spec_e, void *stream);
extern "C" int dfb_apply(dfb_model *m, dfb_state *st, const float *d_spec, const float *d_m, const float *d_coefs,
                         int64_t B, int64_t T, float *d_spec_e, void *stream) {
    if (m && m->cfg.model_kind == 1 && !m->mask_only)
        return fail(DFB_ERR_UNSUPPORTED, "DeepFilterNet v1 blends with df_alpha: use dfb_model_forward_full / dfb_enhance");
    return apply_impl(m, st, d_spec, d_m, d_coefs, nullptr, B, T, d_spec_e, stream);
}
static int apply_impl(dfb_model *m, dfb_state *st, const float *d_spec, const float *d_m, const float *d_coefs, const float *d_alpha,
                      int64_t B, int64_t T, float *d_spec_e, void *stream) {
    if (!m || !st || !d_spec || !d_m || !d_coefs || !d_spec_e) return fail(DFB_ERR_INVALID, "null argument");
    if (int rcs = check_state(m, st)) return rcs;
    DFB_CUDA(cudaSetDevice(m->device));
    dfb::ApplyParams p{};
    p.spec = (const float2 *)d_spec; p.m = d_m; p.coefs = d_coefs; p.audio = nullptr; p.spec_out = (float2 *)d_spec_e;
    p.Tf = (int)T; p.mode = apply_mode(m); p.nb_df = m->cfg.nb_df; p.order = m->cfg.df_order; p.lookahead = m->cfg.df_lookahead;
    p.alpha = d_alpha;
    apply_options(m, p);
    return launch_apply_synthesis(st, p, B, (cudaStream_t)stream);
}

extern "C" int dfb_model_forward_full(dfb_model *m, dfb_state *st, const float *d_spec, const float *d_feat_erb,
                                      const float *d_feat_spec, int64_t B, int64_t T, float *d_spec_e, float *d_m,
                                      float *d_lsnr, float *d_coefs, float *d_alpha, void *stream) {
    if (!m || !st || !d_spec || !d_feat_erb || !d_feat_spec || !d_spec_e) return fail(DFB_ERR_INVALID, "null argument");
    if (int rcs = check_state(m, st)) return rcs;
    DFB_CUDA(cudaSetDevice(m->device));
    const int64_t M = B * T;
    const int O2 = 2 * m->cfg.df_order;
    if (B <= 0 || T <= 0) return DFB_OK;
    if (B > 65535) return fail(DFB_ERR_INVALID, "more than 65535 streams per call");
    size_t extra = ((size_t)M * m->cfg.nb_erb + (size_t)M * m->cfg.nb_df * O2 + (size_t)M) * 4 + 8192;
    int rc = m->arena.reserve(fwd_plan(m->cfg, (size_t)M, nullptr, nullptr) + extra);
    if (rc) return rc;
    m->arena.reset();
    float *mm = d_m ? d_m : m->arena.take<float>((size_t)M * m->cfg.nb_erb);
    float *cc = d_coefs ? d_coefs : m->arena.take<float>((size_t)M * m->cfg.nb_df * O2);
    float *aa = d_alpha;
    if (!aa && m->cfg.model_kind == 1) aa = m->arena.take<float>((size_t)M);
    rc = forward_impl(m, m->arena, d_feat_erb, d_feat_spec, (int)B, (int)T, mm, cc, d_lsnr, aa, (cudaStream_t)stream);
    if (rc) { m->arena.reset(); return rc; }
    rc = apply_impl(m, st, d_spec, mm, cc, m->cfg.model_kind == 1 ? aa : nullptr, B, T, d_spec_e, stream);
    m->arena.reset();
    return rc;
}

extern "C" int64_t dfb_enhance_out_len(const dfb_state *st, int64_t T, int pad) {
    if (!st) return -1;
    return pad ? T : (T / st->hop) * st->hop;
}

extern "C" int dfb_model_set_max_workspace(dfb_model *m, int64_t bytes) {
    if (!m || bytes <= 0) return fail(DFB_ERR_INVALID, "bad workspace cap");
    m->max_workspace = (size_t)bytes;
    return DFB_OK;
}


struct StreamState {
    int B = 0;
    int64_t a1 = 0, d1 = 0, e1 = 0;
    bool started = false, dnn_started = false;
    float *slab = nullptr;
    float *ana_mem = nullptr;
    float *erb_state = nullptr, *unit_state = nullptr;
    float *h_enc = nullptr, *h_erb = nullptr, *h_df = nullptr;
    float *t_spec = nullptr, *t_fe = nullptr, *t_fs = nullptr;
    float *t_m = nullptr, *t_c = nullptr;
    float *t_l = nullptr;
    float *t_dec = nullptr;
    int n_feat = 0, n_mc = 0, n_dec = 0;
};
constexpr int kMcTail = 6;

struct ChunkGeom { int Lmax, lag, Hf; };
static ChunkGeom chunk_geom(const dfb_model_config &c) {
    ChunkGeom g;
    g.Lmax = c.conv_lookahead > c.df_lookahead ? c.conv_lookahead : c.df_lookahead;
    g.lag = c.model_kind != 3 ? c.df_lookahead : 0;
    g.Hf = kHalo + g.Lmax;
    return g;
}

constexpr int kStateArrays = 13;
struct StateLayout { int64_t off[kStateArrays], row_off[kStateArrays], row_floats; int layers[kStateArrays], per_row[kStateArrays]; };

static size_t state_floats(const dfb_model_config &c, const dfb_state *st, int B, size_t off[16], StateLayout *lay = nullptr) {
    const ChunkGeom g = chunk_geom(c);
    const int E = c.nb_erb, Fd = c.nb_df, O2 = 2 * c.df_order, F = st->tb.F, ED = E / 4 * kCh;
    size_t n = 0;
    if (lay) lay->row_floats = 0;
    auto add = [&](int i, int layers, int per_row) {
        off[i] = n;
        if (lay) {
            lay->off[i] = (int64_t)n; lay->layers[i] = layers; lay->per_row[i] = per_row;
            lay->row_off[i] = lay->row_floats;
            lay->row_floats += (int64_t)layers * per_row;
        }
        n += ((size_t)layers * B * per_row + 63) & ~size_t(63);
    };
    add(0, 1, st->hop); add(1, 1, E); add(2, 1, Fd);
    add(3, c.enc_gru_layers, c.emb_hidden); add(4, c.erb_gru_layers, c.emb_hidden); add(5, c.df_gru_layers, c.df_hidden);
    add(6, 1, g.Hf * 2 * F); add(7, 1, g.Hf * E); add(8, 1, g.Hf * 2 * Fd);
    add(9, 1, kMcTail * E); add(10, 1, kMcTail * Fd * O2);
    add(11, 1, c.conv_kt > 1 ? kHalo * ED : 0);
    add(12, 1, kMcTail);
    return n;
}
static void state_bind(StreamState &S, float *base, const size_t off[16], int B) {
    S.B = B; S.slab = base;
    S.ana_mem = base + off[0]; S.erb_state = base + off[1]; S.unit_state = base + off[2];
    S.h_enc = base + off[3]; S.h_erb = base + off[4]; S.h_df = base + off[5];
    S.t_spec = base + off[6]; S.t_fe = base + off[7]; S.t_fs = base + off[8];
    S.t_m = base + off[9]; S.t_c = base + off[10]; S.t_dec = base + off[11]; S.t_l = base + off[12];
    S.a1 = S.d1 = S.e1 = 0; S.started = S.dnn_started = false; S.n_feat = S.n_mc = S.n_dec = 0;
}

static int save_tail(cudaStream_t s, const float *buf, int T, size_t fe, int n, float *tail, int cap, int B) {
    if (n <= 0) return DFB_OK;
    DFB_CUDA(cudaMemcpy2DAsync(tail + (size_t)(cap - n) * fe, sizeof(float) * fe * cap, buf + (size_t)(T - n) * fe, sizeof(float) * fe * T,
                               sizeof(float) * fe * n, B, cudaMemcpyDeviceToDevice, s));
    return DFB_OK;
}
static int load_tail(cudaStream_t s, float *buf, int T, size_t fe, int n, const float *tail, int cap, int dst_t, int B) {
    if (n <= 0) return DFB_OK;
    DFB_CUDA(cudaMemcpy2DAsync(buf + (size_t)dst_t * fe, sizeof(float) * fe * T, tail + (size_t)(cap - n) * fe, sizeof(float) * fe * cap,
                               sizeof(float) * fe * n, B, cudaMemcpyDeviceToDevice, s));
    return DFB_OK;
}

static size_t chunk_bytes_per_stream(const dfb_model_config &c, const dfb_state *st, int Tw) {
    const ChunkGeom g = chunk_geom(c);
    const int E = c.nb_erb, Fd = c.nb_df, O2 = 2 * c.df_order, F = st->tb.F;
    return (size_t)(Tw + g.Lmax) * (2 * F + E + 2 * Fd) * 4 + (size_t)Tw * (E + (size_t)Fd * O2 + 2) * 4 + fwd_plan(c, (size_t)Tw, nullptr, nullptr) +
           16384;
}

struct ChunkIO {
    const float *audio; int64_t audio_T, audio_stride;
    int64_t audio_frame0;
    const float *init_mem;
    float *out; int64_t out_stride, out_len;
    int64_t out_sample0;
    float atten_lim;
    const float *lsnr_th;
    const RaggedRow *rows = nullptr;
    int nb = 0;
    const LinkRow *links = nullptr;
    int reduce = 0;
    const int64_t *first = nullptr;
    const SlotCtl *ctl = nullptr;
    int64_t lsnr_from = -1;
    float *lsnr_out = nullptr;
};

__global__ void k_lsnr_out(const float *__restrict__ ll, int mcT, float *__restrict__ out, int64_t n_out, int64_t f0, int64_t w0,
                           int t_first, int Te, const RaggedRow *__restrict__ rows, const int64_t *__restrict__ first, int64_t from,
                           int hop) {
    const int b = blockIdx.y;
    const int64_t j = (int64_t)blockIdx.x * blockDim.x + threadIdx.x;
    if (j >= n_out) return;
    int64_t o = (int64_t)b * n_out;
    int te = Te;
    if (rows) {
        te = min(te, (int)(rows[b].Tf - w0));
        o = rows[b].out_off / hop;
    }
    int64_t t0 = max(t_first, stream_first(first, b, w0));
    if (from - w0 > t0) t0 = from - w0;
    const int64_t t = f0 + j - w0;
    if (t >= t0 && t < te) out[o + j] = ll[(int64_t)b * mcT + t];
}

static int run_chunk(dfb_model *m, dfb_state *st, StreamState &S, const ChunkIO &io, int64_t a1n, int64_t d1n, int64_t e1n,
                     cudaStream_t s, int lane = 0, bool pipelined = false) {
    Arena &arena = lane ? m->arena1 : m->arena;
    dfb_model::Lane &L = m->lanes[lane], &P = m->lanes[lane ^ 1];
    const bool have_prev = pipelined && S.started;
    if (have_prev) DFB_CUDA(cudaStreamWaitEvent(s, P.ev_fork, 0));
    const dfb_model_config &c = m->cfg;
    const ChunkGeom g = chunk_geom(c);
    const int B = io.nb > 0 ? io.nb : S.B, E = c.nb_erb, Fd = c.nb_df, O2 = 2 * c.df_order, F = st->tb.F, hop = st->hop;
    const int64_t W0 = S.d1 > kHalo ? S.d1 - kHalo : 0;
    const int Rc = (int)(S.d1 - W0), Tw = (int)(d1n - W0), Tsb = Tw + g.Lmax;
    const int n_hist = (int)(S.a1 - W0);
    const int n_new = (int)(a1n - S.a1), Tv = (int)(a1n - W0);
    if (Tw < Rc || n_hist < 0 || n_hist > S.n_feat || Tv > Tsb || Tsb <= 0)
        return fail(DFB_ERR_INVALID, "inconsistent chunk geometry");
    const bool run_dnn = d1n > S.d1;
    int rc;
// ... 1037 lines not shown
```

deepfilternet_b200/csrc/dfb_tc.cu:

```cuda
#include <cooperative_groups.h>
#include <atomic>
#include <map>
#include <mutex>
#include <cuda.h>
#include <cuda_bf16.h>

#include "dfb_common.cuh"
#include "dfb_dwpw.cuh"
#include "dfb_ptx.cuh"

namespace dfb {

constexpr int kBxBM = 128, kBxBN = 128, kBxBK = 64, kBxStages = 3, kBxThreads = 288;
constexpr int kBxBox = 128 * 128;

struct BxSmem {
    alignas(1024) unsigned char x[kBxStages][2][kBxBox];
    alignas(1024) unsigned char w[kBxStages][2][kBxBox];
    alignas(8) uint64_t full[kBxStages];
    uint64_t empty[kBxStages];
};

__global__ void __launch_bounds__(kBxThreads, 1)
k_gemm_bf16x3(const __grid_constant__ CUtensorMap tmXhi, const __grid_constant__ CUtensorMap tmXlo,
// ... 344 lines not shown
        {
            const uint32_t src = sb + kCvRawOff + (uint32_t)half * 16384u + (uint32_t)r * 128u;
            float4 xs[8];
#pragma unroll
            for (int c = 0; c < 8; c++) xs[c] = lds128(src + (uint32_t)((c ^ (r & 7)) << 4));
#pragma unroll
            for (int c = 0; c < 8; c++) {
                float4 x = xs[c];
                if (zero) x = make_float4(0.f, 0.f, 0.f, 0.f);
                uint32_t h0, l0, h1, l1;
                bf16x2_split(x.x, x.y, h0, l0);
                bf16x2_split(x.z, x.w, h1, l1);
                const int cq = half * 8 + c;
                const uint32_t off = sb + sw128_off(r, cq >> 1) + (cq & 1) * 8;
                sts64(off, h0, h1);
                sts64(off + 16384, l0, l1);
            }
        }
        fence_proxy_async();
        __syncthreads();
        if (tid == 0 && f + 1 < f_end) load_bin(f + 1);
        {
            float acc[1][8][4];
#pragma unroll
            for (int nt = 0; nt < 8; nt++)
#pragma unroll
                for (int c = 0; c < 4; c++) acc[0][nt][c] = 0.f;
            warp_mma_sw128_k64<1>(sb, sb + 16384, sb + kCvW, sb + kCvW + 8192, warp * 16, 0, acc);
#pragma unroll
            for (int nt = 0; nt < 8; nt++)
#pragma unroll
                for (int e = 0; e < 4; e++) {
                    const int n = 8 * nt + 2 * (lane & 3) + (e & 1), g = n >> 5, j = n & 31;
                    const int rr = warp * 16 + (lane >> 2) + 8 * (e >> 1);
                    if (j < NY)
                        asm volatile("st.shared.f32 [%0], %1;" ::"r"(sb + kCvYs + (uint32_t)(rr * kCvYld + g * NY + j) * 4u), "f"(acc[0][nt][e]) : "memory");
                }
        }
        __syncthreads();
        if (tid < 128) {
            const int t = r0 + tid;
            if (tid >= KTP - 1 && tid < KTP - 1 + kCvOut && t < p.T) {
                float z[O2];
#pragma unroll
                for (int g = 0; g < 2; g++)
#pragma unroll
                    for (int o = 0; o < ORDER; o++) {
                        float a = 0.f;
#pragma unroll
                        for (int dt = 0; dt < KTP; dt++) {
                            float y;
                            asm volatile("ld.shared.f32 %0, [%1];" : "=f"(y) : "r"(sb + kCvYs + (uint32_t)((tid - (KTP - 1) + dt) * kCvYld + g * NY + dt * ORDER + o) * 4u));
                            a += y;
                        }
                        z[g * ORDER + o] = a;
                    }
                float outv[O2];
#pragma unroll
                for (int qo = 0; qo < O2; qo++) {
                    float a;
                    asm volatile("ld.shared.f32 %0, [%1];" : "=f"(a) : "r"(s_w2 + 4 * (O2 * O2 + qo)));
#pragma unroll
                    for (int k = 0; k < O2; k++) {
                        float w;
                        asm volatile("ld.shared.f32 %0, [%1];" : "=f"(w) : "r"(s_w2 + 4 * (k * O2 + qo)));
                        a = fmaf(z[k], w, a);
                    }
                    outv[qo] = fmaxf(a, 0.f);
                }
                float *dst = p.coefs + (((int64_t)b * p.T + t) * p.Fd + f) * O2;
#pragma unroll
                for (int qo = 0; qo < O2; qo += 2) *reinterpret_cast<float2 *>(dst + qo) = make_float2(outv[qo], outv[qo + 1]);
            }
        }
    }
}

namespace cg = cooperative_groups;

constexpr int kGtU = 32, kGtRows = 3 * kGtU;
template <int NS, int HH>
struct GtCfg {
    static constexpr int kC = HH / kGtU;
    static constexpr int kKS = HH / 128;
    static constexpr int kMmaWarps = 6 * kKS;
    static constexpr int kGateThreads = 16 * NS;
    static constexpr int kThreads = kGateThreads > 32 * kMmaWarps ? kGateThreads : 32 * kMmaWarps;
    static constexpr int kLbo = (NS / 8) * 256;
    static constexpr int kSbo = 256;
    static constexpr int kPlane = 128;
    static constexpr int kPiece = 4 * kLbo;
    static constexpr int kBuf = (HH / 8) * kLbo;
    static constexpr int kPreLd = NS + 1;
};

template <int NS, int HH>
struct GruTcSmem {
    alignas(1024) unsigned char h[2][GtCfg<NS, HH>::kBuf];
    alignas(128) unsigned char wlo[kGtRows * HH * 2];
    float pre[GtCfg<NS, HH>::kKS][kGtRows][GtCfg<NS, HH>::kPreLd];
    alignas(8) uint64_t bar_h[2];
};

struct GruTcParams {
    const float *xproj;
    const float *whh;
    const float *bhh;
    const float *res;
    float *hout;
    unsigned short *hout_hi, *hout_lo;
    int planes_res;
    const float *h0;
    float *hT;
    int t0, Ts;
    int B, T, Bc;
    long long *dbg;
    unsigned char *xbuf;
    const int64_t *first;
    int64_t w0;
};

template <int NS, int HH, int XG>
__global__ void __launch_bounds__(GtCfg<NS, HH>::kThreads, 1) k_gru_tc(GruTcParams p) {
    using Cfg = GtCfg<NS, HH>;
    constexpr int kGtThreads = Cfg::kThreads, kGtH = HH, kGtC = Cfg::kC, NT = NS / 8;
    extern __shared__ __align__(1024) unsigned char tc_smem_raw[];
    GruTcSmem<NS, HH> &sm = *reinterpret_cast<GruTcSmem<NS, HH> *>(((uintptr_t)tc_smem_raw + 1023) & ~uintptr_t(1023));
    cg::cluster_group cluster = cg::this_cluster();
    const int rank = (int)cluster.block_rank();
    const int group = blockIdx.x / kGtC;
    const int b0 = group * p.Bc;
    const int nb = min(p.Bc, p.B - b0);
    const int tid = threadIdx.x, warp = tid >> 5, lane = tid & 31;
    const int H = kGtH, T = p.T;
    for (int i = tid; i < (int)sizeof(sm.h) / 16; i += kGtThreads) reinterpret_cast<uint4 *>(&sm.h[0][0])[i] = make_uint4(0, 0, 0, 0);
    if (tid == 0) {
        mbar_init(&sm.bar_h[0], XG ? 1 : 2);
        mbar_init(&sm.bar_h[1], XG ? 1 : 2);
        fence_barrier_init();
    }
    if (p.h0) {
        __syncthreads();
        for (int i = tid; i < nb * (kGtH / 2); i += kGtThreads) {
            const int s = i / (kGtH / 2), gu = (i - s * (kGtH / 2)) * 2;
            const float2 hv = *reinterpret_cast<const float2 *>(p.h0 + (int64_t)(b0 + s) * kGtH + gu);
            unsigned short h0b, l0b, h1b, l1b;
            bf16_split(hv.x, h0b, l0b);
            bf16_split(hv.y, h1b, l1b);
            const uint32_t off = (uint32_t)((gu >> 3) * Cfg::kLbo + (s >> 3) * Cfg::kSbo + (s & 7) * 16 + (gu & 7) * 2);
            *reinterpret_cast<uint32_t *>(sm.h[0] + off) = h0b | (uint32_t)h1b << 16;
            *reinterpret_cast<uint32_t *>(sm.h[0] + off + Cfg::kPlane) = l0b | (uint32_t)l1b << 16;
        }
    }
    const bool mma_warp = warp < Cfg::kMmaWarps;
    const int mt = warp % 6, kq = warp / 6;
    uint32_t wa[8][4];
    const uint32_t wlo = smem_u32(sm.wlo);
    if (mma_warp) {
#pragma unroll
        for (int ks = 0; ks < 8; ks++)
#pragma unroll
            for (int e = 0; e < 4; e++) {
                const int rho = 16 * mt + (lane >> 2) + 8 * (e & 1), k = 128 * kq + 16 * ks + 2 * (lane & 3) + 8 * (e >> 1);
                const int gate = rho / kGtU, u = rho - gate * kGtU;
                const float2 w = *reinterpret_cast<const float2 *>(p.whh + ((int64_t)gate * H + rank * kGtU + u) * H + k);
                uint32_t hi, lo;
                bf16x2_split(w.x, w.y, hi, lo);
                wa[ks][e] = hi;
                asm volatile("st.shared.b32 [%0], %1;" ::"r"(wlo + (uint32_t)rho * (HH * 2) + ((((k >> 3) ^ (rho & 7))) << 4) + (k & 7) * 2),
                             "r"(lo) : "memory");
            }
    }
    fence_proxy_async();
    __syncthreads();
    cluster.sync();
    const uint32_t step_bytes = (uint32_t)((kGtC - (XG ? 0 : 1)) * Cfg::kPiece);

    const int up = tid & 15, s = tid >> 4;
    const bool gate_thread = tid < Cfg::kGateThreads;
    const bool active = gate_thread && s < nb;
    const int gu = rank * kGtU + 2 * up;
    float hprev0 = 0.f, hprev1 = 0.f;
    float2 bhr = make_float2(0.f, 0.f), bhz = bhr, bhn = bhr;
    int t_first = 0;
    if (active) {
        t_first = stream_first(p.first, b0 + s, p.w0) - p.t0;
        if (p.h0) {
            const float2 hv = *reinterpret_cast<const float2 *>(p.h0 + (int64_t)(b0 + s) * H + gu);
            hprev0 = hv.x; hprev1 = hv.y;
        }
        bhr = *reinterpret_cast<const float2 *>(p.bhh + gu);
        bhz = *reinterpret_cast<const float2 *>(p.bhh + H + gu);
        bhn = *reinterpret_cast<const float2 *>(p.bhh + 2 * H + gu);
    }
    const uint32_t hoff = (uint32_t)((gu >> 3) * Cfg::kLbo + (s >> 3) * Cfg::kSbo + (s & 7) * 16 + (gu & 7) * 2);
    const uint32_t piece0 = (uint32_t)(rank * Cfg::kPiece);
    const bool dbg_on = p.dbg && blockIdx.x == 0 && tid == 0;
    const int mat = lane >> 3, rr = lane & 7;
    for (int t = 0; t < T; t++) {
        const int cur = t & 1;
        if (dbg_on) p.dbg[t * 8 + 0] = clock64();
        if (tid == 0 && t + 1 < T) mbar_expect_tx(&sm.bar_h[cur ^ 1], step_bytes);
        float2 xr = make_float2(0.f, 0.f), xz = xr, xn = xr;
        if (active) {
            const float *xp = p.xproj + ((int64_t)(b0 + s) * p.Ts + p.t0 + t) * (3 * H) + gu;
            xr = *reinterpret_cast<const float2 *>(xp);
            xz = *reinterpret_cast<const float2 *>(xp + H);
            xn = *reinterpret_cast<const float2 *>(xp + 2 * H);
            if (t + 3 < T && (up & 7) == 0) {
                const float *xq = xp + 3 * (3 * H);
                asm volatile("prefetch.global.L2 [%0];" ::"l"(xq));
                asm volatile("prefetch.global.L2 [%0];" ::"l"(xq + H));
                asm volatile("prefetch.global.L2 [%0];" ::"l"(xq + 2 * H));
            }
        }
        if (t > 0) mbar_wait(&sm.bar_h[cur], (uint32_t)(((t - 1) >> 1) & 1));
        if (dbg_on) p.dbg[t * 8 + 1] = clock64();
        if (mma_warp) {
            float acc[NT][4];
#pragma unroll
            for (int n = 0; n < NT; n++) acc[n][0] = acc[n][1] = acc[n][2] = acc[n][3] = 0.f;
            const uint32_t hb = smem_u32(sm.h[cur]);
#pragma unroll
            for (int ks = 0; ks < 8; ks++) {
                const int k = 128 * kq + 16 * ks;
                uint32_t al[4];
                {
                    const int r = 16 * mt + rr + ((mat & 1) << 3);
                    ldsm_x4(wlo + (uint32_t)r * (HH * 2) + ((((k >> 3) + (mat >> 1)) ^ (r & 7)) << 4), al);
                }
#pragma unroll
                for (int n = 0; n < NT; n++) {
                    uint32_t b[4];
                    ldsm_x4(hb + (uint32_t)(((k >> 3) + (mat & 1)) * Cfg::kLbo + n * Cfg::kSbo + (mat >> 1) * Cfg::kPlane + rr * 16), b);
                    mma_bf16x3(acc[n], wa[ks], al, b[0], b[1], b[2], b[3]);
                }
            }
#pragma unroll
            for (int n = 0; n < NT; n++)
#pragma unroll
                for (int e = 0; e < 4; e++)
                    sm.pre[kq][16 * mt + (lane >> 2) + 8 * (e >> 1)][8 * n + 2 * (lane & 3) + (e & 1)] = acc[n][e];
        }
        __syncthreads();
        if (dbg_on) p.dbg[t * 8 + 2] = clock64();
        uint32_t vhi = 0, vlo = 0;
        if (active) {
            const int u0 = 2 * up;
            float a[6];
#pragma unroll
            for (int g = 0; g < 3; g++) {
                float s0 = 0.f, s1 = 0.f;
#pragma unroll
                for (int q = 0; q < Cfg::kKS; q++) { s0 += sm.pre[q][g * kGtU + u0][s]; s1 += sm.pre[q][g * kGtU + u0 + 1][s]; }
                a[2 * g] = s0; a[2 * g + 1] = s1;
            }
            const float r0 = gt_sigmoid(xr.x + a[0] + bhr.x), r1 = gt_sigmoid(xr.y + a[1] + bhr.y);
            const float z0 = gt_sigmoid(xz.x + a[2] + bhz.x), z1 = gt_sigmoid(xz.y + a[3] + bhz.y);
            const float n0 = gt_tanh(xn.x + r0 * (a[4] + bhn.x)), n1 = gt_tanh(xn.y + r1 * (a[5] + bhn.y));
            hprev0 = (1.f - z0) * n0 + z0 * hprev0;
            hprev1 = (1.f - z1) * n1 + z1 * hprev1;
            if (t < t_first) hprev0 = hprev1 = 0.f;
            unsigned short h0, l0, h1, l1;
            bf16_split(hprev0, h0, l0);
            bf16_split(hprev1, h1, l1);
            vhi = h0 | (uint32_t)h1 << 16;
            vlo = l0 | (uint32_t)l1 << 16;
            if (t + 1 < T) {
                if (XG) {
                    unsigned char *xp = p.xbuf + ((size_t)(group * 2 + (cur ^ 1)) * kGtC + rank) * Cfg::kPiece + (hoff - piece0);
                    *reinterpret_cast<uint32_t *>(xp) = vhi;
                    *reinterpret_cast<uint32_t *>(xp + Cfg::kPlane) = vlo;
                } else {
                    *reinterpret_cast<uint32_t *>(sm.h[cur ^ 1] + hoff) = vhi;
                    *reinterpret_cast<uint32_t *>(sm.h[cur ^ 1] + hoff + Cfg::kPlane) = vlo;
                }
            }
        }
        if (dbg_on) p.dbg[t * 8 + 3] = clock64();
        if (t + 1 < T) { if (XG) fence_proxy_async_global(); else fence_proxy_async(); }
        __syncthreads();
        if (t + 1 < T) {
            if (XG) {
                if (tid == 0) {
                    const unsigned char *xp = p.xbuf + ((size_t)(group * 2 + (cur ^ 1)) * kGtC + rank) * Cfg::kPiece;
                    bulk_load_multicast(smem_u32(sm.h[cur ^ 1]) + piece0, xp, Cfg::kPiece, smem_u32(&sm.bar_h[cur ^ 1]),
                                        (uint16_t)((1u << kGtC) - 1u));
                }
            } else if (lane == 0) {
                const uint32_t src = smem_u32(sm.h[cur ^ 1]) + piece0;
                for (int j = warp; j < kGtC - 1; j += kGtThreads / 32) {
                    const int peer = j + (j >= rank ? 1 : 0);
                    dsmem_bulk_copy(mapa_u32(src, peer), src, Cfg::kPiece, mapa_u32(smem_u32(&sm.bar_h[cur ^ 1]), peer));
                }
                if (warp == 0) mbar_arrive(&sm.bar_h[cur ^ 1]);
            }
        }
        if (dbg_on) p.dbg[t * 8 + 4] = clock64();
        if (active) {
            const int64_t o = ((int64_t)(b0 + s) * p.Ts + p.t0 + t) * H + gu;
            float2 ov = make_float2(hprev0, hprev1);
            if (p.hT && t + 1 == T) *reinterpret_cast<float2 *>(p.hT + (int64_t)(b0 + s) * H + gu) = ov;
            if (p.res) { const float2 rv = *reinterpret_cast<const float2 *>(p.res + o); ov.x += rv.x; ov.y += rv.y; }
            *reinterpret_cast<float2 *>(p.hout + o) = ov;
            if (p.hout_hi) {
                if (p.planes_res && p.res) bf16x2_split(ov.x, ov.y, vhi, vlo);
                *reinterpret_cast<uint32_t *>(p.hout_hi + o) = vhi;
                *reinterpret_cast<uint32_t *>(p.hout_lo + o) = vlo;
            }
        }
    }
    cluster.sync();
}

static unsigned char *gru_xbuf(cudaStream_t s, size_t bytes) {
    struct Ent { unsigned char *p = nullptr; size_t cap = 0; };
    static std::mutex mu;
    static std::map<std::pair<int, cudaStream_t>, Ent> pool;
    int dev = 0;
    cudaGetDevice(&dev);
    std::lock_guard<std::mutex> lk(mu);
    Ent &e = pool[{dev, s}];
    if (e.cap < bytes) {
        if (e.p) { cudaDeviceSynchronize(); cudaFree(e.p); e.p = nullptr; e.cap = 0; }
        const size_t want = (bytes + (1u << 20)) & ~size_t((1u << 20) - 1);
        if (cudaMalloc(&e.p, want) != cudaSuccess) { e.p = nullptr; return nullptr; }
        e.cap = want;
    }
    return e.p;
}

template <int NS, int HH, int XG>
static int gru_tc_config(cudaLaunchConfig_t &cfg, cudaLaunchAttribute (&at)[1]) {
    using Cfg = GtCfg<NS, HH>;
    static PerDeviceOnce attr_once;
    const int smem = (int)sizeof(GruTcSmem<NS, HH>) + 1024;
    if (auto once_guard = attr_once.first()) {
        if (Cfg::kC > 8) DFB_CUDA(cudaFuncSetAttribute(k_gru_tc<NS, HH, XG>, cudaFuncAttributeNonPortableClusterSizeAllowed, 1));
        DFB_CUDA(cudaFuncSetAttribute(k_gru_tc<NS, HH, XG>, cudaFuncAttributeMaxDynamicSharedMemorySize, smem));
    }
    cfg = cudaLaunchConfig_t{};
    cfg.blockDim = dim3(Cfg::kThreads);
    cfg.dynamicSmemBytes = smem;
    at[0].id = cudaLaunchAttributeClusterDimension;
    at[0].val.clusterDim.x = Cfg::kC; at[0].val.clusterDim.y = 1; at[0].val.clusterDim.z = 1;
    cfg.attrs = at; cfg.numAttrs = 1;
    return DFB_OK;
}

template <int NS, int HH, int XG>
static int gru_tc_max_clusters(int *out) {
    static std::atomic<int> cached[64];
    int dev = 0;
    DFB_CUDA(cudaGetDevice(&dev));
    int n = cached[dev & 63].load(std::memory_order_relaxed);
    if (n <= 0) {
        cudaLaunchConfig_t cfg;
        cudaLaunchAttribute at[1];
        int rc = gru_tc_config<NS, HH, XG>(cfg, at);
        if (rc) return rc;
        cfg.gridDim = dim3((unsigned)GtCfg<NS, HH>::kC);
        DFB_CUDA(cudaOccupancyMaxActiveClusters(&n, k_gru_tc<NS, HH, XG>, &cfg));
        cached[dev & 63].store(n, std::memory_order_relaxed);
    }
    *out = n;
    return DFB_OK;
}

template <int NS, int HH, int XG>
static int launch_gru_tc_n(cudaStream_t s, GruTcParams p) {
    using Cfg = GtCfg<NS, HH>;
    cudaLaunchConfig_t cfg;
    cudaLaunchAttribute at[1];
    int rc = gru_tc_config<NS, HH, XG>(cfg, at);
    if (rc) return rc;
    p.Bc = NS;
    const int ngroups = (p.B + NS - 1) / NS;
    cfg.gridDim = dim3((unsigned)(ngroups * Cfg::kC));
    cfg.stream = s;
    if (XG) {
        p.xbuf = gru_xbuf(s, (size_t)ngroups * 2 * Cfg::kC * Cfg::kPiece);
        if (!p.xbuf) return fail(DFB_ERR_OOM, "GRU exchange scratch");
    }
    DFB_PROF(HH == 256 ? "k_gru_tc" : "k_gru_tc512", s);
    DFB_CUDA(cudaLaunchKernelEx(&cfg, k_gru_tc<NS, HH, XG>, p));
    g_launches.fetch_add(1, std::memory_order_relaxed);
    return DFB_OK;
}

int launch_gru_tc(cudaStream_t s, const float *xproj, const float *whh, const float *bhh, const float *res, float *hout,
                  unsigned short *hout_hi, unsigned short *hout_lo, int B, int T, long long *dbg, int wide, int planes_res,
                  const GruWindow *w, int H) {
    GruTcParams p{xproj, whh, bhh, res, hout, hout_hi, hout_lo, planes_res, w ? w->h0 : nullptr, w ? w->hT : nullptr,
                  w ? w->t0 : 0, w ? w->Ts : T, B, T, 0, dbg};
    p.first = w ? w->first : nullptr;
    p.w0 = w ? w->w0 : 0;
    static const int force = getenv("DFB_GRU_NS") ? atoi(getenv("DFB_GRU_NS")) : 0;
    static const int xg = getenv("DFB_GRU_XG") ? atoi(getenv("DFB_GRU_XG")) : 7;
    if (H == 512) return (xg & 1) ? launch_gru_tc_n<16, 512, 1>(s, p) : launch_gru_tc_n<16, 512, 0>(s, p);
    if (H != 256) return fail(DFB_ERR_UNSUPPORTED, "tensor-core recurrence: hidden size %d", H);
    const bool use32 = force ? force == 32 : ((wide && B > 64) || B >= 256);
    static const int no48 = getenv("DFB_GRU_NO48") ? atoi(getenv("DFB_GRU_NO48")) : 0;
    if (use32 && !force && !no48) {
        int wave = 0, rc = gru_tc_max_clusters<32, 256, 1>(&wave);
        if (rc) return rc;
        if (B > wave * 32) return launch_gru_tc_n<48, 256, 1>(s, p);
    }
    if (use32 && (xg & 2)) return launch_gru_tc_n<32, 256, 1>(s, p);
    if (!use32 && (xg & 4)) return launch_gru_tc_n<16, 256, 1>(s, p);
    return use32 ? launch_gru_tc_n<32, 256, 0>(s, p) : launch_gru_tc_n<16, 256, 0>(s, p);
}

int cached_map_f32_sw128(CUtensorMap *out, const void *base, int64_t rows, int64_t cols, int64_t ld, int box_rows);

int launch_df_convp_tc(cudaStream_t s, const float *c0, const float *w_sw, const float *w2, const float *bias, float *coefs, int B, int T,
                       int Fd, const int64_t *first, int64_t w0) {
    if ((int64_t)B * T >= (int64_t(1) << 31) - 256 || B > 65535) return fail(DFB_ERR_UNSUPPORTED, "df pathway conv: batch too large for one launch");
    CUtensorMap mc;
    int rc;
    if ((rc = cached_map_f32_sw128(&mc, c0, (int64_t)B * T, (int64_t)Fd * kCh, (int64_t)Fd * kCh, 128))) return rc;
    const int smem = 1024 + (int)kCvTail + 512 + 64;
    static PerDeviceOnce attr_once;
    if (auto once_guard = attr_once.first())
        DFB_CUDA(cudaFuncSetAttribute(k_df_convp_tc<5, 5>, cudaFuncAttributeMaxDynamicSharedMemorySize, smem));
    CvParams p{w_sw, w2, bias, coefs, T, Fd, first, w0};
    dim3 grid((unsigned)((Fd + kCvBins - 1) / kCvBins), (unsigned)((T + kCvOut - 1) / kCvOut), (unsigned)B);
    DFB_PROF("k_df_convp_tc", s);
    k_df_convp_tc<5, 5><<<grid, kCvThreads, smem, s>>>(mc, p);
    DFB_LAUNCH_CHECK();
    return DFB_OK;
}

int cached_map_bf16(CUtensorMap *out, const void *base, int64_t rows, int64_t cols, int64_t ld, int box_rows);

int launch_gemm_bf16x3(cudaStream_t s, const void *x_hi, const void *x_lo, int64_t ldx, const void *w_hi, const void *w_lo,
                       const float *bias, float *y, int64_t ldy, int64_t M, int N, int K) {
    if (N % kBxBN || K % kBxBK || (ldx % 8) || M <= 0 || ldy % 2 || ((uintptr_t)w_hi & 15) || ((uintptr_t)w_lo & 15))
        return fail(DFB_ERR_UNSUPPORTED, "bf16x3 GEMM shape M=%lld N=%d K=%d", (long long)M, N, K);
    const int nslices = N / kBxBN;
    const int64_t ntiles = (M + kBxBM - 1) / kBxBM;
    if (ntiles * nslices > 0x7fffffff) return fail(DFB_ERR_UNSUPPORTED, "bf16x3 GEMM: M = %lld", (long long)M);
    CUtensorMap mxh, mxl, mwh, mwl;
    int rc;
    if ((rc = cached_map_bf16(&mxh, x_hi, M, K, ldx, kBxBM)) || (rc = cached_map_bf16(&mxl, x_lo, M, K, ldx, kBxBM)) ||
        (rc = cached_map_bf16(&mwh, w_hi, N, K, K, kBxBN)) || (rc = cached_map_bf16(&mwl, w_lo, N, K, K, kBxBN)))
        return rc;
    static PerDeviceOnce attr_once;
    const int smem = (int)sizeof(BxSmem) + 1024;
    if (auto once_guard = attr_once.first()) DFB_CUDA(cudaFuncSetAttribute(k_gemm_bf16x3, cudaFuncAttributeMaxDynamicSharedMemorySize, smem));
    DFB_PROF("k_gemm_bf16x3[gru_proj]", s);
    k_gemm_bf16x3<<<(unsigned)(ntiles * nslices), kBxThreads, smem, s>>>(mxh, mxl, mwh, mwl, bias, y, ldy, (int)M, K, nslices);
    DFB_LAUNCH_CHECK();
    return DFB_OK;
}

}
```

Before: 59240.

## Fuse df_conv1 depthwise/pointwise conv with df_fc_emb grouped linear into one kernel

Adds a TMA-pipelined warp-specialized kernel that runs the strided depthwise conv, the pointwise conv with ReLU and the grouped df_fc_emb linear in one pass. The intermediate c1 activation stays in registers and shared memory and is never written to global memory, and one launch is removed. Several fp32 intermediate outputs (GRU hidden, gl outputs) are also skipped when bf16 planes suffice, which cuts global writes. The risks are heavy shared-memory use at one block per SM, and a fixed grid split between feature slices and row tiles that may underuse the SMs.

Measured after the change: 64810 (median of 6 runs). 9.4% higher.

```diff
diff --git a/deepfilternet_b200/csrc/dfb_common.cuh b/deepfilternet_b200/csrc/dfb_common.cuh
--- a/deepfilternet_b200/csrc/dfb_common.cuh
+++ b/deepfilternet_b200/csrc/dfb_common.cuh
@@ -179,6 +179,10 @@
                  const float *res, int64_t ldr, float *y, int64_t ldy, unsigned short *y_hi, unsigned short *y_lo, int64_t ldp,
                  int64_t M, int G, int Ig, int Hg, int act, float oscale, float ooffset);
 bool gl_bx_geometry(int G, int Ig, int Hg, int *gpc_out, int *hgp_out, int *stages_out);
+bool df_emb_geometry(int Fd, int G, int Ig, int Hg, int kt, int *s_out, int *stages_out);
+int launch_df_emb(cudaStream_t s, const float *c0, int64_t M, int T, int Fd, int kt, const float *dw, const float *bias,
+                  const float *pw_sw, const float *w_img, int G, int Ig, int Hg, const float *res, int64_t ldr,
+                  unsigned short *y_hi, unsigned short *y_lo, int64_t ldp, const int64_t *first, int64_t w0);
 int launch_df_convp_tc(cudaStream_t s, const float *c0, const float *w_sw, const float *w2, const float *bias, float *coefs, int B, int T,
                        int Fd, const int64_t *first = nullptr, int64_t w0 = 0);
 int launch_to_planes(cudaStream_t s, const float *x, int64_t ldx, int64_t M, int K, unsigned short *hi, unsigned short *lo);
diff --git a/deepfilternet_b200/csrc/dfb_gl.cu b/deepfilternet_b200/csrc/dfb_gl.cu
--- a/deepfilternet_b200/csrc/dfb_gl.cu
+++ b/deepfilternet_b200/csrc/dfb_gl.cu
@@ -6,6 +6,7 @@
 #include <tuple>
 
 #include "dfb_common.cuh"
+#include "dfb_dwpw.cuh"
 #include "dfb_ptx.cuh"
 
 namespace dfb {
@@ -152,6 +153,228 @@
             if (c < nch)
                 gl_store_chunk(p, c, g0, cpg, mrow, lane, acc[c][0][0], acc[c][0][1], acc[c][0][2], acc[c][0][3], acc[c][1][0],
                                acc[c][1][1], acc[c][1][2], acc[c][1][3]);
+    }
+}
+
+constexpr int kDeThreads = 288, kDeMaxStages = 6, kDeMaxChunks = 4;
+constexpr uint32_t kDeBin = 32768;
+
+struct DfEmbParams {
+    const float *dw;
+    const float *bias;
+    const float *pw_sw;
+    const unsigned short *w_img;
+    const float *res; int64_t ldr;
+    unsigned short *y_hi, *y_lo; int64_t ldp;
+    int M, T, G, Ig, Hg, Hgp, S, stages;
+    float oscale, ooffset;
+    const int64_t *first;
+    int64_t w0;
+};
+
+template <int KT>
+__global__ void __launch_bounds__(kDeThreads, 1)
+k_dwpw_gl(const __grid_constant__ CUtensorMap tmC0, const __grid_constant__ DfEmbParams p) {
+    extern __shared__ __align__(1024) unsigned char de_smem_raw[];
+    const uint32_t sb = (smem_u32(de_smem_raw) + 1023u) & ~1023u;
+    const int warp = threadIdx.x >> 5, lane = threadIdx.x & 31;
+    constexpr int RT = 128 - (KT - 1);
+    const int ntiles = (p.M + RT - 1) / RT;
+    const int j0 = blockIdx.x * p.S;
+    const int f_lo = j0 > 0 ? 2 * j0 - 1 : 0, f_hi = 2 * (j0 + p.S);
+    const int gps = p.S * kCh / p.Ig, cpg = p.Hgp / 16, nch = gps * cpg;
+    const int g0 = j0 * kCh / p.Ig;
+    const uint32_t gbytes = (uint32_t)p.Ig * p.Hgp * 2;
+    const uint32_t wplane = gbytes * gps;
+    const uint32_t lbo = (uint32_t)(p.Hgp / 8) * 128u;
+    const uint32_t s_c0 = sb;
+    const uint32_t s_pw = s_c0 + (uint32_t)p.stages * kDeBin;
+    const uint32_t s_w = s_pw + 2u * kCh * 128u;
+    const uint32_t s_bias = s_w + 2 * wplane;
+    const uint32_t s_dw = s_bias + 256u;
+    const uint32_t s_bar = (s_dw + KT * 3 * kCh * 4u + 127u) & ~127u;
+    const uint32_t b_full = s_bar, b_empty = s_bar + 8 * kDeMaxStages, b_w = b_empty + 8 * kDeMaxStages;
+    if (threadIdx.x == 0) {
+        for (int s = 0; s < p.stages; s++) { mbar_init_a(b_full + 8 * s, 1); mbar_init_a(b_empty + 8 * s, 8); }
+        mbar_init_a(b_w, 1);
+        fence_barrier_init();
+        mbar_expect_tx_a(b_w, 2u * kCh * 128u + 2 * wplane);
+        bulk_load(s_pw, p.pw_sw, 2u * kCh * 128u, b_w);
+        const unsigned char *src = reinterpret_cast<const unsigned char *>(p.w_img);
+        bulk_load(s_w, src + (size_t)g0 * gbytes, wplane, b_w);
+        bulk_load(s_w + wplane, src + (size_t)p.G * gbytes + (size_t)g0 * gbytes, wplane, b_w);
+    }
+    if (threadIdx.x < kCh / 4) sts128(s_bias + threadIdx.x * 16, __ldg(reinterpret_cast<const float4 *>(p.bias) + threadIdx.x));
+    for (int i = threadIdx.x; i < KT * 3 * kCh / 4; i += kDeThreads) sts128(s_dw + i * 16, __ldg(reinterpret_cast<const float4 *>(p.dw) + i));
+    __syncthreads();
+    if (warp == 8) {
+        if (lane == 0) {
+            tma_prefetch_desc(&tmC0);
+            int it = 0;
+            for (int tile = blockIdx.y; tile < ntiles; tile += gridDim.y) {
+                const int row0 = tile * RT - (KT - 1);
+                for (int f = f_lo; f < f_hi; f++, it++) {
+                    const int s = it % p.stages, n = it / p.stages;
+                    if (n > 0) mbar_wait_a(b_empty + 8 * s, (uint32_t)((n - 1) & 1));
+                    mbar_expect_tx_a(b_full + 8 * s, kDeBin);
+                    const uint32_t dst = s_c0 + (uint32_t)s * kDeBin;
+                    asm volatile(
+                        "cp.async.bulk.tensor.2d.shared::cluster.global.mbarrier::complete_tx::bytes [%0], [%1, {%2, %3}], [%4];"
+                        ::"r"(dst), "l"((uint64_t)&tmC0), "r"(f * kCh), "r"(row0), "r"(b_full + 8 * s) : "memory");
+                    asm volatile(
+                        "cp.async.bulk.tensor.2d.shared::cluster.global.mbarrier::complete_tx::bytes [%0], [%1, {%2, %3}], [%4];"
+                        ::"r"(dst + kDeBin / 2), "l"((uint64_t)&tmC0), "r"(f * kCh + 32), "r"(row0), "r"(b_full + 8 * s) : "memory");
+                }
+            }
+        }
+        return;
+    }
+    const int g = lane >> 2, q = lane & 3, mat = lane >> 3, rr = lane & 7;
+    mbar_wait_a(b_w, 0);
+    int it = 0;
+    for (int tile = blockIdx.y; tile < ntiles; tile += gridDim.y, it += f_hi - f_lo) {
+        const int row0 = tile * RT - (KT - 1);
+        bool tap_ok[2][KT];
+#pragma unroll
+        for (int rs = 0; rs < 2; rs++) {
+            const int r = warp * 16 + g + 8 * rs, m = row0 + r;
+#pragma unroll
+            for (int dt = 0; dt < KT; dt++) tap_ok[rs][dt] = true;
+            if (KT > 1) {
+                const int b = m >= 0 && m < p.M ? m / p.T : 0, t = m - b * p.T;
+                const int t_first = stream_first(p.first, b, p.w0);
+#pragma unroll
+                for (int dt = 0; dt < KT; dt++) tap_ok[rs][dt] = r - (KT - 1) + dt >= 0 && t - (KT - 1 - dt) >= t_first;
+            }
+        }
+        float gacc[kDeMaxChunks][2][4];
+#pragma unroll
+        for (int c = 0; c < kDeMaxChunks; c++)
+#pragma unroll
+            for (int e = 0; e < 8; e++) gacc[c][e >> 2][e & 3] = 0.f;
+        for (int jj = 0; jj < p.S; jj++) {
+            const int j = j0 + jj;
+            uint32_t slot[3];
+#pragma unroll
+            for (int df = 0; df < 3; df++) {
+                const int f = 2 * j - 1 + df;
+                const int i = it + (f < f_lo ? 0 : f - f_lo);
+                slot[df] = s_c0 + (uint32_t)(i % p.stages) * kDeBin;
+                if (f >= f_lo) mbar_wait_a(b_full + 8 * (i % p.stages), (uint32_t)((i / p.stages) & 1));
+            }
+            uint32_t ah[4][4], al[4][4];
+#pragma unroll
+            for (int ks = 0; ks < 4; ks++)
+#pragma unroll
+                for (int h = 0; h < 2; h++) {
+                    const int ch = 16 * ks + 8 * h + 2 * q;
+                    const uint32_t cbase = (uint32_t)(ch >> 5) * (kDeBin / 2) + (uint32_t)(ch & 3) * 4u;
+                    const int chunk = (ch & 31) >> 2;
+#pragma unroll
+                    for (int rs = 0; rs < 2; rs++) {
+                        const int r = warp * 16 + g + 8 * rs;
+                        float2 acc = make_float2(0.f, 0.f);
+#pragma unroll
+                        for (int dt = 0; dt < KT; dt++) {
+                            if (!tap_ok[rs][dt]) continue;
+                            const int rb = r - (KT - 1) + dt;
+                            const uint32_t o = cbase + (uint32_t)rb * 128u + (uint32_t)((chunk ^ (rb & 7)) << 4);
+#pragma unroll
+                            for (int df = 0; df < 3; df++) {
+                                if (df == 0 && j == 0) continue;
+                                float2 x;
+                                asm volatile("ld.shared.v2.f32 {%0, %1}, [%2];" : "=f"(x.x), "=f"(x.y) : "r"(slot[df] + o));
+                                float2 w;
+                                asm volatile("ld.shared.v2.f32 {%0, %1}, [%2];" : "=f"(w.x), "=f"(w.y) : "r"(s_dw + 4u * ((dt * 3 + df) * kCh + ch)));
+                                acc.x = fmaf(x.x, w.x, acc.x);
+                                acc.y = fmaf(x.y, w.y, acc.y);
+                            }
+                        }
+                        bf16x2_split(acc.x, acc.y, ah[ks][rs + 2 * h], al[ks][rs + 2 * h]);
+                    }
+                }
+            __syncwarp();
+            if (lane == 0) {
+                for (int f = 2 * j - 1; f <= 2 * j + (jj + 1 == p.S ? 1 : 0); f++)
+                    if (f >= f_lo) mbar_arrive_a(b_empty + 8 * ((it + f - f_lo) % p.stages));
+            }
+            float acc[8][4];
+#pragma unroll
+            for (int nt = 0; nt < 8; nt++)
+#pragma unroll
+                for (int e = 0; e < 4; e++) acc[nt][e] = 0.f;
+#pragma unroll
+            for (int ks = 0; ks < 4; ks++)
+#pragma unroll
+                for (int np = 0; np < 4; np++) {
+                    const int n = 16 * np + rr + ((mat >> 1) << 3);
+                    const uint32_t o = sw128_off(n, 2 * ks + (mat & 1));
+                    uint32_t bh[4], bl[4];
+                    ldsm_x4(s_pw + o, bh);
+                    ldsm_x4(s_pw + 8192 + o, bl);
+                    mma_bf16x3(acc[2 * np], ah[ks], al[ks], bh[0], bh[1], bl[0], bl[1]);
+                    mma_bf16x3(acc[2 * np + 1], ah[ks], al[ks], bh[2], bh[3], bl[2], bl[3]);
+                }
+            uint32_t ch_[4][4], cl_[4][4];
+#pragma unroll
+            for (int nt = 0; nt < 8; nt++) {
+                const int c = 8 * nt + 2 * q;
+                float b0, b1;
+                asm volatile("ld.shared.v2.f32 {%0, %1}, [%2];" : "=f"(b0), "=f"(b1) : "r"(s_bias + 4 * c));
+#pragma unroll
+                for (int rs = 0; rs < 2; rs++)
+                    bf16x2_split(fmaxf(acc[nt][2 * rs] + b0, 0.f), fmaxf(acc[nt][2 * rs + 1] + b1, 0.f), ch_[nt >> 1][rs + 2 * (nt & 1)],
+                                 cl_[nt >> 1][rs + 2 * (nt & 1)]);
+            }
+#pragma unroll
+            for (int kk = 0; kk < 4; kk++) {
+                const int col = jj * kCh + kk * 16;
+                const int gl = col / p.Ig, kq = (col - gl * p.Ig) >> 4;
+                const uint32_t wa = s_w + (uint32_t)gl * gbytes + (uint32_t)(2 * kq + (mat & 1)) * lbo + (uint32_t)rr * 16u;
+#pragma unroll
+                for (int c = 0; c < kDeMaxChunks; c++) {
+                    const int cg = c - gl * cpg;
+                    if (c >= nch || cg < 0 || cg >= cpg) continue;
+                    const uint32_t o = wa + (uint32_t)(2 * cg + (mat >> 1)) * 128u;
+                    uint32_t bh[4], bl[4];
+                    ldsm_x4(o, bh);
+                    ldsm_x4(o + wplane, bl);
+                    mma_bf16x3(gacc[c][0], ch_[kk], cl_[kk], bh[0], bh[1], bl[0], bl[1]);
+                    mma_bf16x3(gacc[c][1], ch_[kk], cl_[kk], bh[2], bh[3], bl[2], bl[3]);
+                }
+            }
+        }
+        const int64_t mrow = (int64_t)row0 + warp * 16 + g;
+        const int64_t mmin = (int64_t)tile * RT;
+#pragma unroll
+        for (int c = 0; c < kDeMaxChunks; c++) {
+            if (c >= nch) continue;
+            const int gl = c / cpg;
+#pragma unroll
+            for (int jh = 0; jh < 2; jh++) {
+                const int n = (c - gl * cpg) * 16 + jh * 8 + 2 * q;
+                if (n >= p.Hg) continue;
+                const int64_t col = (int64_t)(g0 + gl) * p.Hg + n;
+                float2 rv[2];
+#pragma unroll
+                for (int rs = 0; rs < 2; rs++) {
+                    const int64_t m = mrow + 8 * rs;
+                    rv[rs] = (p.res && m >= mmin && m < p.M) ? *reinterpret_cast<const float2 *>(p.res + m * p.ldr + col) : make_float2(0.f, 0.f);
+                }
+#pragma unroll
+                for (int rs = 0; rs < 2; rs++) {
+                    const int64_t m = mrow + 8 * rs;
+                    if (m < mmin || m >= p.M) continue;
+                    float2 x;
+                    x.x = gx_act(gacc[c][jh][2 * rs], 1) * p.oscale + p.ooffset + rv[rs].x;
+                    x.y = gx_act(gacc[c][jh][2 * rs + 1], 1) * p.oscale + p.ooffset + rv[rs].y;
+                    uint32_t hv, lv;
+                    bf16x2_split(x.x, x.y, hv, lv);
+                    *reinterpret_cast<uint32_t *>(p.y_hi + m * p.ldp + col) = hv;
+                    *reinterpret_cast<uint32_t *>(p.y_lo + m * p.ldp + col) = lv;
+                }
+            }
+        }
     }
 }
 
@@ -299,4 +522,53 @@
     return DFB_OK;
 }
 
-}
+bool df_emb_geometry(int Fd, int G, int Ig, int Hg, int kt, int *s_out, int *stages_out) {
+    if ((kt != 1 && kt != 2) || Fd % 2 || Ig % 16 || Hg % 4 || G < 1 || G * Ig != Fd / 2 * kCh) return false;
+    int S = 1;
+    while ((S * kCh) % Ig) S++;
+    const int Hgp = (Hg + 15) / 16 * 16;
+    if ((Fd / 2) % S || (S * kCh / Ig) * (Hgp / 16) > kDeMaxChunks) return false;
+    const int fixed = 1024 + 2 * kCh * 128 + S * kCh * Hgp * 4 + 256 + kt * 3 * kCh * 4 + 128 + 2 * 8 * kDeMaxStages + 8;
+    int stages = (227 * 1024 - fixed) / (int)kDeBin;
+    if (stages > kDeMaxStages) stages = kDeMaxStages;
+    if (stages < 3) return false;
+    *s_out = S; *stages_out = stages;
+    return true;
+}
+
+int launch_df_emb(cudaStream_t s, const float *c0, int64_t M, int T, int Fd, int kt, const float *dw, const float *bias,
+                  const float *pw_sw, const float *w_img, int G, int Ig, int Hg, const float *res, int64_t ldr,
+                  unsigned short *y_hi, unsigned short *y_lo, int64_t ldp, const int64_t *first, int64_t w0) {
+    int S = 0, stages = 0;
+    if (!df_emb_geometry(Fd, G, Ig, Hg, kt, &S, &stages) || M <= 0 || M > 0x7fffffff - 256 || T <= 0 || M % T ||
+        (res && ((ldr % 2) || ((uintptr_t)res & 7))) || (ldp % 2) || ((uintptr_t)y_hi & 3) || ((uintptr_t)y_lo & 3) ||
+        ((uintptr_t)c0 & 15) || ((uintptr_t)w_img & 15) || ((uintptr_t)pw_sw & 15))
+        return fail(DFB_ERR_UNSUPPORTED, "df_conv1 + df_fc_emb kernel: shape G %d Ig %d Hg %d kt %d", G, Ig, Hg, kt);
+    CUtensorMap mc;
+    int rc;
+    if ((rc = cached_map_f32_sw128(&mc, c0, M, (int64_t)Fd * kCh, (int64_t)Fd * kCh, 128))) return rc;
+    const int Hgp = (Hg + 15) / 16 * 16;
+    DfEmbParams p{dw, bias, pw_sw, reinterpret_cast<const unsigned short *>(w_img), res, ldr, y_hi, y_lo, ldp,
+                  (int)M, T, G, Ig, Hg, Hgp, S, stages, 1.f, 0.f, first, w0};
+    const int smem = 1024 + stages * (int)kDeBin + 2 * kCh * 128 + S * kCh * Hgp * 4 + 256 + kt * 3 * kCh * 4 + 128 + 2 * 8 * kDeMaxStages + 8;
+    static PerDeviceOnce attr_once;
+    if (auto once_guard = attr_once.first()) {
+        DFB_CUDA(cudaFuncSetAttribute(k_dwpw_gl<1>, cudaFuncAttributeMaxDynamicSharedMemorySize, 227 * 1024));
+        DFB_CUDA(cudaFuncSetAttribute(k_dwpw_gl<2>, cudaFuncAttributeMaxDynamicSharedMemorySize, 227 * 1024));
+    }
+    int dev = 0, sms = 0;
+    DFB_CUDA(cudaGetDevice(&dev));
+    DFB_CUDA(cudaDeviceGetAttribute(&sms, cudaDevAttrMultiProcessorCount, dev));
+    const int slices = Fd / 2 / S, rt = 128 - (kt - 1);
+    const int ntiles = (int)((M + rt - 1) / rt);
+    int groups = sms / slices;
+    if (groups < 1) groups = 1;
+    if (groups > ntiles) groups = ntiles;
+    DFB_PROF("k_dwpw_gl", s);
+    if (kt == 1) k_dwpw_gl<1><<<dim3((unsigned)slices, (unsigned)groups), kDeThreads, smem, s>>>(mc, p);
+    else k_dwpw_gl<2><<<dim3((unsigned)slices, (unsigned)groups), kDeThreads, smem, s>>>(mc, p);
+    DFB_LAUNCH_CHECK();
+    return DFB_OK;
+}
+
+}
diff --git a/deepfilternet_b200/csrc/dfb_model.cu b/deepfilternet_b200/csrc/dfb_model.cu
--- a/deepfilternet_b200/csrc/dfb_model.cu
+++ b/deepfilternet_b200/csrc/dfb_model.cu
@@ -578,7 +578,7 @@
 }
 
 int run_gru(dfb_model *m, cudaStream_t s, const char *name, int layers, int H, int in_dim, const float *res_last, float *y,
-            float *xproj, float *tmp_h, int B, int T, const unsigned short *x_hi, const unsigned short *x_lo,
+            float *xproj, int B, int T, const unsigned short *x_hi, const unsigned short *x_lo,
             unsigned short *pl_hi, unsigned short *pl_lo, int wide, unsigned short *out_hi, unsigned short *out_lo,
             bool *out_planes_ok, const GruChunk *ck) {
     if (out_planes_ok) *out_planes_ok = false;
@@ -600,7 +600,7 @@
             return rc;
         if ((rc = launch_gemm_bf16x3(s, cur_hi, cur_lo, cur_dim, w_hi, w_lo, b_ih, xproj, 3 * H, M, 3 * H, cur_dim))) return rc;
         const bool last = l == layers - 1;
-        float *dst = last ? y : tmp_h;
+        float *dst = last ? y : nullptr;
         float *hs = ck && ck->h ? ck->h + (int64_t)l * ck->Bs * H : nullptr;
         GruWindow gw{ck && ck->have_state ? hs : nullptr, hs, t0, T, ck ? ck->first : nullptr, ck ? ck->w0 : 0};
         unsigned short *hi = last ? out_hi : pl_hi, *lo = last ? out_lo : pl_lo;
@@ -642,9 +642,9 @@
 }
 
 struct FwdBufs {
-    float *e0, *e1, *e2, *e3, *c0, *c1, *emb_in, *emb, *g_a, *g_b, *g_h, *xproj, *dec_emb, *d3, *d2, *d1, *dfc;
+    float *e0, *e1, *e2, *e3, *c0, *c1, *emb_in, *emb, *g_a, *g_b, *xproj, *dec_emb, *d3, *d2, *d1, *dfc;
     unsigned short *ga_hi, *ga_lo, *gh_hi, *gh_lo;
-    float *g_a2, *g_h2, *xproj2, *dfskip;
+    float *g_a2, *xproj2, *dfskip;
     unsigned short *ga2_hi, *ga2_lo, *gh2_hi, *gh2_lo;
     unsigned short *c1_hi, *c1_lo, *embin_hi, *embin_lo, *gb_hi, *gb_lo, *emb_hi, *emb_lo, *dfc_hi, *dfc_lo;
 };
@@ -677,6 +677,14 @@
     return bytes + 4096;
 }
 
+static bool fused_emb_shape(const dfb_model_config &c) {
+    const int Fd = c.nb_df, ED = c.nb_erb / 4 * kCh, I = Fd / 2 * kCh, G = c.g_df_fc_emb, Ge = c.g_enc_in, H = c.emb_hidden;
+    const int emb_in_dim = c.enc_concat ? 2 * ED : ED;
+    int de_s, de_st, gpc, hgp, stg;
+    return c.model_kind != 1 && G > 0 && I % G == 0 && ED % G == 0 && df_emb_geometry(Fd, G, I / G, ED / G, c.conv_kt, &de_s, &de_st) &&
+           Ge > 0 && emb_in_dim % Ge == 0 && H % Ge == 0 && gl_bx_geometry(Ge, emb_in_dim / Ge, H / Ge, &gpc, &hgp, &stg);
+}
+
 static size_t fwd_plan(const dfb_model_config &c, size_t M, Arena *a, FwdBufs *f) {
     if (c.model_kind == 1 && !a) return fwd_plan_v1(c, M, nullptr, nullptr);
     const int E = c.nb_erb, Fd = c.nb_df, H = c.emb_hidden, Hd = c.df_hidden;
@@ -695,13 +703,14 @@
     t.e3 = c.enc_concat ? t.emb_in : take(M * ED);
     t.c0 = take(M * Fd * kCh); t.c1 = take(M * (Fd / 2) * kCh);
     t.emb = take(M * emb_dim);
-    t.g_a = take(M * Hmax); t.g_b = take(M * Hmax); t.g_h = take(M * Hmax);
+    t.g_a = take(M * Hmax); t.g_b = take(M * Hmax);
+    take(M * Hmax);
     t.xproj = take(M * 3 * Hmax);
     t.dec_emb = take(M * ED); t.d3 = take(M * ED); t.d2 = take(M * (E / 2) * kCh);
     t.d1 = take(M * E * kCh); t.dfc = take(M * Hmax);
     t.ga_hi = reinterpret_cast<unsigned short *>(take(M * Hmax / 2)); t.ga_lo = reinterpret_cast<unsigned short *>(take(M * Hmax / 2));
     t.gh_hi = reinterpret_cast<unsigned short *>(take(M * Hmax / 2)); t.gh_lo = reinterpret_cast<unsigned short *>(take(M * Hmax / 2));
-    t.g_a2 = take(M * Hmax); t.g_h2 = take(M * Hmax); t.xproj2 = take(M * 3 * Hmax); t.dfskip = take(M * Hmax);
+    t.g_a2 = take(M * Hmax); take(M * Hmax); t.xproj2 = take(M * 3 * Hmax); t.dfskip = take(M * Hmax);
     t.ga2_hi = reinterpret_cast<unsigned short *>(take(M * Hmax / 2)); t.ga2_lo = reinterpret_cast<unsigned short *>(take(M * Hmax / 2));
     t.gh2_hi = reinterpret_cast<unsigned short *>(take(M * Hmax / 2)); t.gh2_lo = reinterpret_cast<unsigned short *>(take(M * Hmax / 2));
     auto take16 = [&](size_t n) { return reinterpret_cast<unsigned short *>(take((n + 1) / 2)); };
@@ -807,7 +816,27 @@
     m->dbg["d2"] = {f.d2, M * (E / 2) * kCh}; m->dbg["d1"] = {f.d1, M * E * kCh}; m->dbg["dfc"] = {f.dfc, M * Hd};
     m->dbg["g_a"] = {f.g_a, M * (H > Hd ? H : Hd)}; m->dbg["g_b"] = {f.g_b, M * (H > Hd ? H : Hd)};
     m->dbg["xproj"] = {f.xproj, M * 3 * (H > Hd ? H : Hd)};
+    m->dbg["emb_in_hi"] = {reinterpret_cast<const float *>(f.embin_hi), M * emb_in_dim / 2};
+    m->dbg["emb_in_lo"] = {reinterpret_cast<const float *>(f.embin_lo), M * emb_in_dim / 2};
     const int64_t e3_fs = c.enc_concat ? 2 * ED : ED;
+    auto gl_is_bx = [&](const char *wname, int G, int I, int Hh) -> bool {
+        int gpc, hgp, stg;
+        return G > 0 && I % G == 0 && Hh % G == 0 && m->get(std::string(wname) + "_bx") && gl_bx_geometry(G, I / G, Hh / G, &gpc, &hgp, &stg);
+    };
+    const float *emb_w = m->get("enc.df_fc_emb.gl_bx");
+    const bool fused_emb = fused_emb_shape(c);
+    if (fused_emb && (!emb_w || !gl_is_bx("enc.emb_gru.in.gl", c.g_enc_in, emb_in_dim, H)))
+        return fail(DFB_ERR_INVALID, "df_fc_emb / enc.emb_gru.in: tensor-core weight images missing");
+    const bool keep_ga = c.model_kind == 2;
+    float *const enc_ga = gl_is_bx("enc.emb_gru.in.gl", c.g_enc_in, emb_in_dim, H) ? nullptr : f.g_a;
+    float *const erb_ga = !keep_ga && gl_is_bx("erb_dec.emb_gru.in.gl", c.g_erb_in, emb_dim, H) ? nullptr : f.g_a;
+    float *const df_ga = !keep_ga && gl_is_bx("df_dec.df_gru.in.gl", c.g_df_in, emb_dim, Hd) ? nullptr : f.g_a2;
+    float *const enc_gb = c.g_enc_out && gl_is_bx("enc.emb_gru.out.gl", c.g_enc_out, H, ED) ? nullptr : f.g_b;
+    float *const erb_gb = gl_is_bx("erb_dec.emb_gru.out.gl", c.g_erb_out, H, ED) ? nullptr : f.g_b;
+    float *const dfc = c.model_kind != 2 && gl_is_bx("df_dec.df_out.gl", c.g_df_out, Hd, Fd * 2 * c.df_order) ? nullptr : f.dfc;
+    if (!erb_ga) m->dbg.erase("g_a");
+    if (!erb_gb) m->dbg.erase("g_b");
+    if (!dfc) m->dbg.erase("dfc");
     struct Pl { unsigned short *hi, *lo; int64_t ld; bool ok; };
     Pl pl_c1{f.c1_hi, f.c1_lo, (int64_t)Fd / 2 * kCh, false}, pl_embin{f.embin_hi, f.embin_lo, emb_in_dim, false},
        pl_gb{f.gb_hi, f.gb_lo, H, false}, pl_emb{f.emb_hi, f.emb_lo, emb_dim, false}, pl_dfc{f.dfc_hi, f.dfc_lo, Hd, false},
@@ -815,6 +844,7 @@
     auto ensure_planes = [&](cudaStream_t st, const float *x, int64_t ldx, int K, Pl &pl) -> int {
         if (pl.ok) return DFB_OK;
         if (pl.ld != K) return fail(DFB_ERR_INVALID, "plane pitch mismatch");
+        if (!x) return fail(DFB_ERR_INVALID, "planes requested of an activation whose fp32 form was not written");
         int r = launch_to_planes(st, x, ldx, M, K, pl.hi, pl.lo);
         if (!r) pl.ok = true;
         return r;
@@ -836,6 +866,9 @@
                 return r;
             }
         }
+        if (!x || !y)
+            return fail(DFB_ERR_UNSUPPORTED, "grouped linear '%s': the tensor-core kernel cannot take this launch and the fp32 %s "
+                        "the FFMA kernel needs is not written", wname, x ? "output" : "input");
         const bool ffma_planes = yout && yout->ld == ldy;
         r = run_gl(st, x, ldx, w, nullptr, res, ldr, y, ldy, M, G, I, Hh, act, 1.f, 0.f, ffma_planes ? yh : nullptr, ffma_planes ? yl : nullptr);
         if (!r && yout) yout->ok = ffma_planes;
@@ -882,11 +915,13 @@
             DFB_LAUNCH_CHECK();
             DFB_CUDA(cudaEventRecord(L.ev_c0, sa));
         }
-        p = mk(f.c0, Fd, (int64_t)Fd * kCh, f.c1, Fd / 2, (int64_t)Fd / 2 * kCh, c.conv_kt);
-        if ((rc = blk("enc.df_conv1", p))) return rc;
-        p.out = nullptr; p.out_hi = pl_c1.hi; p.out_lo = pl_c1.lo; pl_c1.ok = true;
         m->dbg.erase("c1");
-        if ((rc = run_dwpw<DW_S2>(sa, p, B, pw_sw))) return rc;
+        if (!fused_emb) {
+            p = mk(f.c0, Fd, (int64_t)Fd * kCh, f.c1, Fd / 2, (int64_t)Fd / 2 * kCh, c.conv_kt);
+            if ((rc = blk("enc.df_conv1", p))) return rc;
+            p.out = nullptr; p.out_hi = pl_c1.hi; p.out_lo = pl_c1.lo; pl_c1.ok = true;
+            if ((rc = run_dwpw<DW_S2>(sa, p, B, pw_sw))) return rc;
+        }
         DFB_CUDA(cudaEventRecord(L.ev_join_enc, sa));
         DFB_CUDA(cudaStreamWaitEvent(sl, L.ev_c0, 0));
         const int O2 = 2 * c.df_order;
@@ -915,7 +950,15 @@
     DFB_CUDA(cudaStreamWaitEvent(s, L.ev_join_enc, 0));
     {
         const int I = Fd / 2 * kCh;
-        if (c.enc_concat) {
+        if (fused_emb) {
+            DwPwParams p{};
+            if ((rc = blk("enc.df_conv1", p))) return rc;
+            const int G = c.g_df_fc_emb;
+            rc = launch_df_emb(s, f.c0, M, T, Fd, c.conv_kt, p.dw, p.bias, pw_sw, emb_w, G, I / G, ED / G, c.enc_concat ? nullptr : f.e3,
+                               ED, pl_embin.hi + (c.enc_concat ? ED : 0), pl_embin.lo + (c.enc_concat ? ED : 0), pl_embin.ld, first, W0);
+            if (!rc) pl_embin.ok = true;
+            m->dbg.erase("emb_in");
+        } else if (c.enc_concat) {
             rc = gl(s, "enc.df_fc_emb.gl", f.c1, I, &pl_c1, c.g_df_fc_emb, I, ED, ACT_RELU, nullptr, 0, f.emb_in + ED, emb_in_dim,
                     &pl_embin, ED);
         } else {
@@ -924,14 +967,15 @@
         if (rc) return rc;
     }
     {
-        if ((rc = gl(s, "enc.emb_gru.in.gl", f.emb_in, emb_in_dim, &pl_embin, c.g_enc_in, emb_in_dim, H, ACT_RELU, nullptr, 0, f.g_a, H,
+        if ((rc = gl(s, "enc.emb_gru.in.gl", fused_emb ? nullptr : f.emb_in, emb_in_dim, &pl_embin, c.g_enc_in, emb_in_dim, H, ACT_RELU,
+                     nullptr, 0, enc_ga, H,
                      &pl_ga))) return rc;
-        float *gout = c.g_enc_out ? f.g_b : f.emb;
+        float *gout = c.g_enc_out ? enc_gb : f.emb;
         Pl &pl_gout = c.g_enc_out ? pl_gb : pl_emb;
-        if ((rc = run_gru(m, s, "enc.emb_gru", c.enc_gru_layers, H, H, nullptr, gout, f.xproj, f.g_h, B, T, f.ga_hi, f.ga_lo,
+        if ((rc = run_gru(m, s, "enc.emb_gru", c.enc_gru_layers, H, H, nullptr, gout, f.xproj, B, T, f.ga_hi, f.ga_lo,
                           f.gh_hi, f.gh_lo, 0, pl_gout.hi, pl_gout.lo, &pl_gout.ok, cx ? &ck_enc : nullptr))) return rc;
         if (c.g_enc_out) {
-            if ((rc = gl(s, "enc.emb_gru.out.gl", f.g_b, H, &pl_gb, c.g_enc_out, H, ED, ACT_RELU, nullptr, 0, f.emb, emb_dim, &pl_emb)))
+            if ((rc = gl(s, "enc.emb_gru.out.gl", enc_gb, H, &pl_gb, c.g_enc_out, H, ED, ACT_RELU, nullptr, 0, f.emb, emb_dim, &pl_emb)))
                 return rc;
         }
         if ((rc = ensure_planes(s, f.emb, emb_dim, emb_dim, pl_emb))) return rc;
@@ -959,11 +1003,11 @@
     }
     {
         cudaStream_t s = sa;
-        if ((rc = gl(s, "df_dec.df_gru.in.gl", f.emb, emb_dim, &pl_emb, c.g_df_in, emb_dim, Hd, ACT_RELU, nullptr, 0, f.g_a2, Hd, &pl_ga2)))
+        if ((rc = gl(s, "df_dec.df_gru.in.gl", f.emb, emb_dim, &pl_emb, c.g_df_in, emb_dim, Hd, ACT_RELU, nullptr, 0, df_ga, Hd, &pl_ga2)))
             return rc;
         const float *res = c.model_kind == 2 ? f.g_a2 : (early_skip ? f.dfskip : nullptr);
         if (early_skip) DFB_CUDA(cudaStreamWaitEvent(s, L.ev_skip, 0));
-        if ((rc = run_gru(m, s, "df_dec.df_gru", c.df_gru_layers, Hd, Hd, res, f.dfc, f.xproj2, f.g_h2, B, T, f.ga2_hi, f.ga2_lo,
+        if ((rc = run_gru(m, s, "df_dec.df_gru", c.df_gru_layers, Hd, Hd, res, dfc, f.xproj2, B, T, f.ga2_hi, f.ga2_lo,
                           f.gh2_hi, f.gh2_lo, wide_df, pl_dfc.hi, pl_dfc.lo, &pl_dfc.ok, cx ? &ck_df : nullptr))) return rc;
         if (c.g_df_skip && !early_skip) {
             if ((rc = gl(s, "df_dec.df_skip.gl", f.emb, emb_dim, &pl_emb, c.g_df_skip, emb_dim, Hd, ACT_NONE, f.dfc, Hd, f.dfc, Hd, nullptr)))
@@ -977,18 +1021,18 @@
         }
         const int O2 = 2 * c.df_order;
         DFB_CUDA(cudaStreamWaitEvent(s, L.ev_convp, 0));
-        if ((rc = gl(s, "df_dec.df_out.gl", f.dfc, Hd, &pl_dfc, c.g_df_out, Hd, Fd * O2, ACT_TANH, d_coefs, (int64_t)Fd * O2, d_coefs,
+        if ((rc = gl(s, "df_dec.df_out.gl", dfc, Hd, &pl_dfc, c.g_df_out, Hd, Fd * O2, ACT_TANH, d_coefs, (int64_t)Fd * O2, d_coefs,
                      (int64_t)Fd * O2, nullptr))) return rc;
     }
     DFB_CUDA(cudaEventRecord(L.ev_join, sa));
     {
-        if ((rc = gl(s, "erb_dec.emb_gru.in.gl", f.emb, emb_dim, &pl_emb, c.g_erb_in, emb_dim, H, ACT_RELU, nullptr, 0, f.g_a, H, &pl_ga)))
+        if ((rc = gl(s, "erb_dec.emb_gru.in.gl", f.emb, emb_dim, &pl_emb, c.g_erb_in, emb_dim, H, ACT_RELU, nullptr, 0, erb_ga, H, &pl_ga)))
             return rc;
         const float *res = c.model_kind == 2 ? f.g_a : nullptr;
         pl_gb.ok = false;
-        if ((rc = run_gru(m, s, "erb_dec.emb_gru", c.erb_gru_layers, H, H, res, f.g_b, f.xproj, f.g_h, B, T, f.ga_hi, f.ga_lo,
+        if ((rc = run_gru(m, s, "erb_dec.emb_gru", c.erb_gru_layers, H, H, res, erb_gb, f.xproj, B, T, f.ga_hi, f.ga_lo,
                           f.gh_hi, f.gh_lo, wide_erb, pl_gb.hi, pl_gb.lo, &pl_gb.ok, cx ? &ck_erb : nullptr))) return rc;
-        if ((rc = gl(s, "erb_dec.emb_gru.out.gl", f.g_b, H, &pl_gb, c.g_erb_out, H, ED, ACT_RELU, nullptr, 0, f.dec_emb, ED, nullptr)))
+        if ((rc = gl(s, "erb_dec.emb_gru.out.gl", erb_gb, H, &pl_gb, c.g_erb_out, H, ED, ACT_RELU, nullptr, 0, f.dec_emb, ED, nullptr)))
             return rc;
         if (cx && cx->dec_tail && c.conv_kt > 1) {
             const size_t fb = sizeof(float) * ED;
@@ -1150,7 +1194,7 @@
             const std::string nm = std::string(name) + ".g" + std::to_string(l);
             GruChunk ck{hbase ? hbase + (int64_t)l * B * H : nullptr, false, 0, B, nullptr, 0};
             bool ok = false;
-            int r = run_gru(m, st, nm.c_str(), 1, H, H, nullptr, y[l], xproj, nullptr, B, T, ch, cl, f.scr_hi, f.scr_lo, 0, y_hi[l], y_lo[l], &ok,
+            int r = run_gru(m, st, nm.c_str(), 1, H, H, nullptr, y[l], xproj, B, T, ch, cl, f.scr_hi, f.scr_lo, 0, y_hi[l], y_lo[l], &ok,
                             hbase ? &ck : nullptr);
             if (r) return r;
             ch = y_hi[l]; cl = y_lo[l];
diff --git a/deepfilternet_b200/csrc/dfb_tc.cu b/deepfilternet_b200/csrc/dfb_tc.cu
--- a/deepfilternet_b200/csrc/dfb_tc.cu
+++ b/deepfilternet_b200/csrc/dfb_tc.cu
@@ -670,7 +670,7 @@
             float2 ov = make_float2(hprev0, hprev1);
             if (p.hT && t + 1 == T) *reinterpret_cast<float2 *>(p.hT + (int64_t)(b0 + s) * H + gu) = ov;
             if (p.res) { const float2 rv = *reinterpret_cast<const float2 *>(p.res + o); ov.x += rv.x; ov.y += rv.y; }
-            *reinterpret_cast<float2 *>(p.hout + o) = ov;
+            if (p.hout) *reinterpret_cast<float2 *>(p.hout + o) = ov;
             if (p.hout_hi) {
                 if (p.planes_res && p.res) bf16x2_split(ov.x, ov.y, vhi, vlo);
                 *reinterpret_cast<uint32_t *>(p.hout_hi + o) = vhi;
@@ -759,6 +759,7 @@
 int launch_gru_tc(cudaStream_t s, const float *xproj, const float *whh, const float *bhh, const float *res, float *hout,
                   unsigned short *hout_hi, unsigned short *hout_lo, int B, int T, long long *dbg, int wide, int planes_res,
                   const GruWindow *w, int H) {
+    if (!hout && !hout_hi) return fail(DFB_ERR_INVALID, "tensor-core recurrence: neither an fp32 output nor planes");
     GruTcParams p{xproj, whh, bhh, res, hout, hout_hi, hout_lo, planes_res, w ? w->h0 : nullptr, w ? w->hT : nullptr,
                   w ? w->t0 : 0, w ? w->Ts : T, B, T, 0, dbg};
     p.first = w ? w->first : nullptr;
```
